# noahares/raxtax

Hardware: AMD Instinct MI355X
Metric: classified queries/sec (whole node) (higher is better)
Workload: dtype u32 bit-planes + f64

## Files before the change

include/raxtax_hip.h:

```cpp
#ifndef RAXTAX_HIP_H
#define RAXTAX_HIP_H

#include <stddef.h>
#include <stdint.h>

#ifdef __cplusplus
extern "C" {
#endif

#define RTX_ABI_VERSION 6
#define RTX_NUM_KMERS 65536u
#define RTX_MAX_DEPTH 32u

#define RTX_OK 0
#define RTX_ERR_INVALID (-1)
#define RTX_ERR_HIP (-2)
#define RTX_ERR_NO_DEVICE (-3)
#define RTX_ERR_OOM (-4)
#define RTX_ERR_PARSE (-5)
#define RTX_ERR_DEPTH (-6)
#define RTX_ERR_STATE (-7)
#define RTX_ERR_TOO_LONG (-8)
#define RTX_ERR_SENDER (-9)
#define RTX_RETRY_CHUNK 1

#define RTX_SKIP_EXACT_MATCHES 1u
#define RTX_RAW_CONFIDENCE 2u
#define RTX_TEXT_TSV 4u

#define RTX_Q_OK 0
#define RTX_Q_NO_KMERS 1

#define RTX_Q_ALL_KMERS 2

typedef struct rtx_tree rtx_tree;
typedef struct rtx_index rtx_index;

int rtx_abi_version(void);
const char *rtx_last_error(void);
int rtx_device_count(void);

int rtx_tree_build(uint64_t n, const char *lineage_bytes, const uint64_t *lineage_off,
                   const uint8_t *seq_bytes, const uint64_t *seq_off, rtx_tree **out);
#define RTX_TREE_SKIP_KMER_MAP 1u
int rtx_tree_build_ex(uint64_t n, const char *lineage_bytes, const uint64_t *lineage_off,
                      const uint8_t *seq_bytes, const uint64_t *seq_off, uint32_t flags, rtx_tree **out);
int rtx_tree_parse_reference_fasta(const char *text, uint64_t len, rtx_tree **out);
int rtx_tree_parse_reference_fasta_ex(const char *text, uint64_t len, uint32_t flags, rtx_tree **out);
int rtx_tree_build_kmer_map(rtx_tree *tree);
int rtx_tree_save_bin(const rtx_tree *tree, const char *path);
int rtx_tree_load_bin(const char *path, rtx_tree **out);
void rtx_tree_destroy(rtx_tree *tree);
uint64_t rtx_tree_num_tips(const rtx_tree *tree);
const char *rtx_tree_lineage(const rtx_tree *tree, uint64_t i);
uint64_t rtx_tree_original_index(const rtx_tree *tree, uint64_t i);
int rtx_tree_kmer_csr(const rtx_tree *tree, const uint64_t **offsets, const uint32_t **postings);
uint64_t rtx_tree_exact_matches(const rtx_tree *tree, const uint8_t *seq, uint64_t len,
                                const uint32_t **ids);
uint64_t rtx_tree_exact_matches_batch(const rtx_tree *tree, uint64_t n_queries, const uint8_t *bases,
                                      const uint64_t *base_off, uint64_t *exact_off, uint32_t *exact_ids,
                                      uint64_t ids_cap);
typedef struct {
    uint32_t n_nodes;
    const uint32_t *node_begin;
    const uint32_t *node_end;
    const uint32_t *node_first_child;
    const uint32_t *node_n_children;
    const uint32_t *node_parent;
    const uint8_t *node_type;
} rtx_nodes_view;
int rtx_tree_nodes(const rtx_tree *tree, rtx_nodes_view *out);

typedef struct rtx_queries rtx_queries;
int rtx_queries_parse_fasta(const char *text, uint64_t len, const char *const *skip, uint64_t n_skip,
                            rtx_queries **out);
#define RTX_FASTA_MORE_FOLLOWS 1u
#define RTX_FASTA_NOT_FIRST 2u
uint64_t rtx_fasta_block_end(const char *text, uint64_t len);
int rtx_queries_parse_fasta_block(const char *text, uint64_t len, const char *const *skip, uint64_t n_skip, uint32_t flags,
                                  rtx_queries **out);
void rtx_queries_destroy(rtx_queries *q);
uint64_t rtx_queries_len(const rtx_queries *q);
const char *rtx_queries_label(const rtx_queries *q, uint64_t i);
int rtx_queries_data(const rtx_queries *q, const uint8_t **bases, const uint64_t **base_off);

int rtx_index_create(int device, uint64_t n_refs, const uint64_t *offsets ,
                     const uint32_t *postings, uint32_t n_nodes, const uint32_t *node_begin,
                     const uint32_t *node_end, const uint32_t *node_first_child,
                     const uint32_t *node_n_children, const uint8_t *node_type, rtx_index **out);
int rtx_index_create_shard(int device, uint64_t n_refs_total, uint64_t ref_lo, uint64_t ref_hi,
                           const uint64_t *shard_cuts, uint32_t n_cuts, const uint64_t *offsets,
                           const uint32_t *postings, uint32_t n_nodes, const uint32_t *node_begin,
                           const uint32_t *node_end, const uint32_t *node_first_child,
                           const uint32_t *node_n_children, const uint8_t *node_type, rtx_index **out);
int rtx_index_create_from_sequences(int device, uint64_t n_refs, const uint8_t *seq_bytes, const uint64_t *seq_off,
                                    uint32_t n_nodes, const uint32_t *node_begin, const uint32_t *node_end,
                                    const uint32_t *node_first_child, const uint32_t *node_n_children,
                                    const uint8_t *node_type, rtx_index **out);
int rtx_index_create_from_tree(int device, const rtx_tree *tree, rtx_index **out);
void rtx_index_destroy(rtx_index *index);
uint64_t rtx_index_num_refs(const rtx_index *index);
uint64_t rtx_index_device_bytes(const rtx_index *index);
uint64_t rtx_index_workspace_bytes(const rtx_index *index);
int rtx_index_workspace_parts(const rtx_index *index, uint64_t out[9]);
int rtx_index_set_batch(rtx_index *index, uint32_t sub_batch);
#define RTX_OPT_SUB_BATCH 1
#define RTX_OPT_PROB_MODE 2
#define RTX_OPT_STAGE_TIMING 6
#define RTX_OPT_DEBUG_TAPS 14
#define RTX_OPT_DEVICE_EXACT 15
#define RTX_OPT_CLUSTER 7
#define RTX_OPT_PACKED_COUNTS 8
#define RTX_OPT_HIT_PAIR 11
#define RTX_OPT_TILE_SKIP 10
#define RTX_OPT_LOCATOR 12
#define RTX_OPT_TILE_PRUNE 13
#define RTX_OPT_FINE_BOUNDS 17
#define RTX_OPT_RECORDS 18
#define RTX_OPT_OVERLAP 19
#define RTX_OPT_MIN_SUB_BATCHES 20
#define RTX_OPT_TWO_LEVEL_BOUNDS 21
#define RTX_OPT_PRUNE_SELF_SAMPLE 22
#define RTX_OPT_RUN_AHEAD 23
#define RTX_OPT_DEVICE_TEXT 24
#define RTX_OPT_STRAND 25
#define RTX_OPT_NEAREST 26
#define RTX_NO_REF 0xFFFFFFFFu
#define RTX_OPT_DEREP 27
int rtx_index_set_option(rtx_index *index, int option, uint64_t value);

int rtx_index_self_sample(rtx_index *index, const uint8_t *seq_bytes, const uint64_t *seq_off, uint64_t n_refs, uint32_t n_sample, double *live_fraction);
int rtx_index_prune_verdict(const rtx_index *index, int *pruning, double *live_fraction);
int rtx_index_run_ahead_stats(const rtx_index *index, uint64_t *enqueued_ahead, uint64_t *abandoned);
#define RTX_DEFAULT_SEGMENT_CLASSES 1
#define RTX_DEFAULT_EXACT_HASH_MASK 2
#define RTX_DEFAULT_DEREP_HASH_MASK 3
int rtx_set_default_option(int option, uint64_t value);

typedef struct {
    uint32_t n_queries;
    uint64_t n_rows;
    const uint32_t *t;
    const uint8_t *status;
    const double *global_signal;
    const uint64_t *row_begin;
    const uint32_t *row_count;
    const uint32_t *row_lineage;
    const uint32_t *row_node;
    const uint32_t *row_depth;
    const double *row_conf;
    const double *row_local_signal;
    uint32_t row_conf_stride;
    const uint8_t *row_depth_u8;
    const uint8_t *row_conf_hundredths;
} rtx_result_view;

int rtx_batch_prefetch(rtx_index *index, uint64_t n_queries, const uint8_t *bases, const uint64_t *base_off,
                       const uint32_t *exact_ids, const uint64_t *exact_off);
int rtx_batch_activate(rtx_index *index);
int rtx_pack_bases(const uint8_t *bases, uint64_t n_bases, uint8_t *packed);
int rtx_classify_batch(rtx_index *index, uint64_t n_queries, const uint8_t *bases,
                       const uint64_t *base_off, const uint32_t *exact_ids,
                       const uint64_t *exact_off, uint32_t flags, rtx_result_view *out);
int rtx_index_has_exact_lookup(const rtx_index *index);
int rtx_batch_exact_matches(rtx_index *index, const uint64_t **exact_off , const uint32_t **exact_ids);

int rtx_batch_strands(rtx_index *index, const uint8_t **strand, const uint32_t **peak);
int rtx_revcomp(const uint8_t *in, uint64_t n, uint8_t *out);
int rtx_batch_nearest(rtx_index *index, const uint32_t **nearest, const uint32_t **ties);
int rtx_batch_nearest_time(rtx_index *index, float *ms, uint32_t *launches);

typedef struct {
    uint32_t n_nodes;
    uint32_t cutoff_hundredths;
    uint32_t flags;
    const uint64_t *clade, *direct, *conf_sum;
    uint64_t totals[4];
} rtx_profile_view;
int rtx_index_profile_begin(rtx_index *index, uint32_t cutoff_hundredths, uint32_t flags);
int rtx_index_profile_read(rtx_index *index, rtx_profile_view *out);
int rtx_index_profile_reset(rtx_index *index);
int rtx_index_profile_end(rtx_index *index);
int rtx_index_profile_time(rtx_index *index, float *ms, uint32_t *launches);
int rtx_profile_merge(rtx_profile_view *const *views, uint32_t n, uint64_t *clade, uint64_t *direct, uint64_t *conf_sum, uint64_t totals[4]);
int64_t rtx_profile_format(const rtx_tree *tree, const uint64_t *clade, const uint64_t *direct, const uint64_t *conf_sum,
                           const uint64_t totals[4], uint32_t cutoff_hundredths, char *out, uint64_t cap);

// ... 120 lines not shown
```

raxtax_amd/_lib.py:

```python
from __future__ import annotations

import ctypes as C
from pathlib import Path

import numpy as np

PKG = Path(__file__).resolve().parent
import os as _os

LIB_PATH = Path(_os.environ.get("RTX_LIB_PATH") or PKG / "libraxtax_hip.so")

RTX_MAX_DEPTH = 32
RTX_NUM_KMERS = 65536
RTX_OK = 0
RTX_ERR_INVALID, RTX_ERR_HIP, RTX_ERR_NO_DEVICE, RTX_ERR_OOM = -1, -2, -3, -4
RTX_ERR_PARSE, RTX_ERR_DEPTH, RTX_ERR_STATE, RTX_ERR_TOO_LONG = -5, -6, -7, -8
RTX_SKIP_EXACT_MATCHES = 1
RTX_RAW_CONFIDENCE = 2
RTX_TEXT_TSV = 4
RTX_Q_OK, RTX_Q_NO_KMERS, RTX_Q_ALL_KMERS = 0, 1, 2
RTX_OPT_DEREP = 27
RTX_DEFAULT_DEREP_HASH_MASK = 3
STAGES = ("kmer_extract", "hit_count", "prob_table", "taxon_prefix", "lineage_walk", "tile_bounds", "tile_prune", "exact_match", "order", "pair_union")

# ... 3 lines not shown
u64p = C.POINTER(C.c_uint64)
f64p = C.POINTER(C.c_double)
f32p = C.POINTER(C.c_float)


class NodesView(C.Structure):
    _fields_ = [("n_nodes", C.c_uint32), ("node_begin", u32p), ("node_end", u32p), ("node_first_child", u32p),
                ("node_n_children", u32p), ("node_parent", u32p), ("node_type", u8p)]


class ResultView(C.Structure):
    _fields_ = [("n_queries", C.c_uint32), ("n_rows", C.c_uint64), ("t", u32p), ("status", u8p),
                ("global_signal", f64p), ("row_begin", u64p), ("row_count", u32p), ("row_lineage", u32p), ("row_node", u32p),
                ("row_depth", u32p), ("row_conf", f64p), ("row_local_signal", f64p),
                ("row_conf_stride", C.c_uint32), ("row_depth_u8", u8p), ("row_conf_hundredths", u8p)]


class TextView(C.Structure):
    _fields_ = [("n_queries", C.c_uint64), ("out", C.c_void_p), ("out_off", u64p), ("tsv", C.c_void_p), ("tsv_off", u64p)]


class ProfileView(C.Structure):
    _fields_ = [("n_nodes", C.c_uint32), ("cutoff_hundredths", C.c_uint32), ("flags", C.c_uint32), ("clade", u64p), ("direct", u64p),
                ("conf_sum", u64p), ("totals", C.c_uint64 * 4)]


class RtxError(RuntimeError):
    def __init__(self, code: int, msg: str):
        super().__init__(f"libraxtax_hip error {code}: {msg}")
        self.code = code


_SIGNATURES = {
    "rtx_abi_version": (C.c_int, []),
    "rtx_last_error": (C.c_char_p, []),
    "rtx_device_count": (C.c_int, []),
    "rtx_tree_build": (C.c_int, [C.c_uint64, C.c_char_p, u64p, u8p, u64p, C.POINTER(C.c_void_p)]),
    "rtx_tree_build_ex": (C.c_int, [C.c_uint64, C.c_char_p, u64p, u8p, u64p, C.c_uint32, C.POINTER(C.c_void_p)]),
    "rtx_tree_parse_reference_fasta": (C.c_int, [C.c_char_p, C.c_uint64, C.POINTER(C.c_void_p)]),
    "rtx_tree_parse_reference_fasta_ex": (C.c_int, [C.c_char_p, C.c_uint64, C.c_uint32, C.POINTER(C.c_void_p)]),
    "rtx_tree_build_kmer_map": (C.c_int, [C.c_void_p]),
    "rtx_tree_save_bin": (C.c_int, [C.c_void_p, C.c_char_p]),
    "rtx_tree_load_bin": (C.c_int, [C.c_char_p, C.POINTER(C.c_void_p)]),
    "rtx_tree_destroy": (None, [C.c_void_p]),
    "rtx_tree_num_tips": (C.c_uint64, [C.c_void_p]),
    "rtx_tree_lineage": (C.c_char_p, [C.c_void_p, C.c_uint64]),
    "rtx_tree_original_index": (C.c_uint64, [C.c_void_p, C.c_uint64]),
    "rtx_tree_kmer_csr": (C.c_int, [C.c_void_p, C.POINTER(u64p), C.POINTER(u32p)]),
    "rtx_tree_exact_matches": (C.c_uint64, [C.c_void_p, u8p, C.c_uint64, C.POINTER(u32p)]),
    "rtx_tree_exact_matches_batch": (C.c_uint64, [C.c_void_p, C.c_uint64, u8p, u64p, u64p, u32p, C.c_uint64]),
    "rtx_tree_nodes": (C.c_int, [C.c_void_p, C.POINTER(NodesView)]),
    "rtx_fasta_block_end": (C.c_uint64, [C.c_char_p, C.c_uint64]),
    "rtx_queries_parse_fasta_block": (C.c_int, [C.c_char_p, C.c_uint64, C.POINTER(C.c_char_p), C.c_uint64, C.c_uint32,
                                      C.POINTER(C.c_void_p)]),
    "rtx_queries_parse_fasta": (C.c_int, [C.c_char_p, C.c_uint64, C.POINTER(C.c_char_p), C.c_uint64,
                                          C.POINTER(C.c_void_p)]),
    "rtx_queries_destroy": (None, [C.c_void_p]),
    "rtx_queries_len": (C.c_uint64, [C.c_void_p]),
    "rtx_queries_label": (C.c_char_p, [C.c_void_p, C.c_uint64]),
    "rtx_queries_data": (C.c_int, [C.c_void_p, C.POINTER(u8p), C.POINTER(u64p)]),
    "rtx_index_create": (C.c_int, [C.c_int, C.c_uint64, u64p, u32p, C.c_uint32, u32p, u32p, u32p, u32p, u8p,
                                   C.POINTER(C.c_void_p)]),
    "rtx_index_create_shard": (C.c_int, [C.c_int, C.c_uint64, C.c_uint64, C.c_uint64, u64p, C.c_uint32, u64p, u32p, C.c_uint32,
                                        u32p, u32p, u32p, u32p, u8p, C.POINTER(C.c_void_p)]),
    "rtx_shard_begin": (C.c_int, [C.c_void_p, u32p, u32p]),
    "rtx_shard_count": (C.c_int, [C.c_void_p, C.c_uint32, C.c_uint32]),
    "rtx_shard_bounds": (C.c_int, [C.c_void_p, C.c_uint32, C.c_uint32]),
    "rtx_shard_prunes": (C.c_int, [C.c_void_p]),
    "rtx_shard_prob": (C.c_int, [C.c_void_p, C.c_uint32]),
    "rtx_shard_walk": (C.c_int, [C.c_void_p, C.c_uint32, C.c_void_p]),
    "rtx_shard_info": (C.c_int, [C.c_void_p, u64p, u64p, u32p, u32p, u32p]),
    "rtx_device_buffer": (C.c_int, [C.c_void_p, C.c_int, C.POINTER(C.c_void_p), u64p]),
    "rtx_shard_buffer": (C.c_int, [C.c_void_p, C.c_uint32, C.c_int, C.POINTER(C.c_void_p), u64p]),
    "rtx_shard_rehist": (C.c_int, [C.c_void_p, C.c_uint32]),
    "rtx_index_stream": (C.c_int, [C.c_void_p, C.POINTER(C.c_void_p)]),
    "rtx_index_create_from_sequences": (C.c_int, [C.c_int, C.c_uint64, u8p, u64p, C.c_uint32, u32p, u32p, u32p, u32p, u8p,
                                                 C.POINTER(C.c_void_p)]),
    "rtx_index_create_from_tree": (C.c_int, [C.c_int, C.c_void_p, C.POINTER(C.c_void_p)]),
    "rtx_index_destroy": (None, [C.c_void_p]),
    "rtx_index_num_refs": (C.c_uint64, [C.c_void_p]),
    "rtx_index_device_bytes": (C.c_uint64, [C.c_void_p]),
    "rtx_index_workspace_bytes": (C.c_uint64, [C.c_void_p]),
    "rtx_index_workspace_parts": (C.c_int, [C.c_void_p, u64p]),
    "rtx_index_set_batch": (C.c_int, [C.c_void_p, C.c_uint32]),
    "rtx_set_default_option": (C.c_int, [C.c_int, C.c_uint64]),
    "rtx_index_set_option": (C.c_int, [C.c_void_p, C.c_int, C.c_uint64]),
    "rtx_index_self_sample": (C.c_int, [C.c_void_p, C.c_void_p, C.c_void_p, C.c_uint64, C.c_uint32, C.POINTER(C.c_double)]),
    "rtx_index_prune_verdict": (C.c_int, [C.c_void_p, C.POINTER(C.c_int), C.POINTER(C.c_double)]),
    "rtx_index_run_ahead_stats": (C.c_int, [C.c_void_p, C.POINTER(C.c_uint64), C.POINTER(C.c_uint64)]),
    "rtx_classify_batch": (C.c_int, [C.c_void_p, C.c_uint64, u8p, u64p, u32p, u64p, C.c_uint32,
                                     C.POINTER(ResultView)]),
    "rtx_index_has_exact_lookup": (C.c_int, [C.c_void_p]),
    "rtx_batch_exact_matches": (C.c_int, [C.c_void_p, C.POINTER(u64p), C.POINTER(u32p)]),
    "rtx_batch_upload": (C.c_int, [C.c_void_p, C.c_uint64, u8p, u64p, u32p, u64p]),
    "rtx_batch_run": (C.c_int, [C.c_void_p, C.c_uint32]),
    "rtx_batch_sync": (C.c_int, [C.c_void_p]),
    "rtx_batch_download": (C.c_int, [C.c_void_p, C.POINTER(ResultView)]),
    "rtx_batch_download_then_run": (C.c_int, [C.c_void_p, C.POINTER(ResultView), C.c_uint32]),
    "rtx_index_text_setup": (C.c_int, [C.c_void_p, C.c_void_p, C.c_uint32]),
    "rtx_batch_prefetch_labels": (C.c_int, [C.c_void_p, C.c_uint64, C.POINTER(C.c_char_p)]),
    "rtx_batch_text": (C.c_int, [C.c_void_p, C.POINTER(TextView)]),
    "rtx_batch_stage_times": (C.c_int, [C.c_void_p, f32p, u32p]),
    "rtx_batch_work": (C.c_int, [C.c_void_p, u64p, u64p, u64p]),
    "rtx_batch_prob_work": (C.c_int, [C.c_void_p, u64p, u64p]),
    "rtx_batch_work_split": (C.c_int, [C.c_void_p, u64p, u64p]),
    "rtx_debug_kmers": (C.c_int, [C.c_void_p, C.c_uint64, u16p, u32p]),
    "rtx_debug_hit_counts": (C.c_int, [C.c_void_p, C.c_uint64, u16p]),
    "rtx_debug_prob_table": (C.c_int, [C.c_void_p, C.c_uint64, f64p, f64p]),
    "rtx_debug_pruned_prob_table": (C.c_int, [C.c_void_p, C.c_uint64, f64p, f64p, u32p]),
    "rtx_debug_probs": (C.c_int, [C.c_void_p, C.c_uint64, f64p]),
    "rtx_debug_order": (C.c_int, [C.c_void_p, u32p]),
    "rtx_debug_tile_bounds": (C.c_int, [C.c_void_p, C.c_uint64, u16p]),
    "rtx_debug_prune_stats": (C.c_int, [C.c_void_p, u64p]),
    "rtx_debug_run_counts": (C.c_int, [C.c_void_p, C.c_uint64, u16p, u8p, u32p, u32p, u32p]),
    "rtx_debug_run_mode": (C.c_int, [C.c_void_p, C.c_uint64, u32p]),
    "rtx_batch_last_sub_batch": (C.c_int, [C.c_void_p, u64p, u32p]),
    "rtx_batch_classes": (C.c_int, [C.c_void_p, u32p, u64p]),
    "rtx_debug_prune_detail": (C.c_int, [C.c_void_p, C.c_uint64, u32p]),
    "rtx_debug_evaluate": (C.c_int, [C.c_void_p, f64p, C.POINTER(ResultView)]),
    "rtx_result_pack": (C.c_int64, [C.POINTER(ResultView), u8p, C.c_uint64]),
    "rtx_records_format": (C.c_int64, [C.c_void_p, u8p, C.c_uint64, C.POINTER(C.c_char_p), u32p, C.c_uint32, C.c_char_p, C.c_uint64, u64p, C.c_uint32]),
    "rtx_format_query": (C.c_int64, [C.c_void_p, C.POINTER(ResultView), C.c_uint64, C.c_char_p, u8p, C.c_uint64,
                                     u32p, C.c_uint64, C.c_uint32, C.c_char_p, C.c_uint64, C.c_char_p, C.c_uint64,
                                     C.POINTER(C.c_int64)]),
    "rtx_raxtax": (C.c_int, None),
    "rtx_raxtax_multi": (C.c_int, None),
    "rtx_raxtax_multi_ex": (C.c_int, None),
    "rtx_batch_strands": (C.c_int, [C.c_void_p, C.POINTER(u8p), C.POINTER(u32p)]),
    "rtx_revcomp": (C.c_int, [u8p, C.c_uint64, u8p]),
    "rtx_raxtax_multi_ex2": (C.c_int, None),
    "rtx_batch_nearest": (C.c_int, [C.c_void_p, C.POINTER(u32p), C.POINTER(u32p)]),
    "rtx_batch_nearest_time": (C.c_int, [C.c_void_p, C.POINTER(C.c_float), C.POINTER(C.c_uint32)]),
    "rtx_index_profile_begin": (C.c_int, [C.c_void_p, C.c_uint32, C.c_uint32]),
    "rtx_index_profile_read": (C.c_int, [C.c_void_p, C.POINTER(ProfileView)]),
    "rtx_index_profile_reset": (C.c_int, [C.c_void_p]),
    "rtx_index_profile_end": (C.c_int, [C.c_void_p]),
    "rtx_index_profile_time": (C.c_int, [C.c_void_p, C.POINTER(C.c_float), C.POINTER(C.c_uint32)]),
    "rtx_profile_merge": (C.c_int, [C.POINTER(C.POINTER(ProfileView)), C.c_uint32, u64p, u64p, u64p, u64p]),
    "rtx_profile_format": (C.c_int64, [C.c_void_p, u64p, u64p, u64p, u64p, C.c_uint32, C.c_char_p, C.c_uint64]),
    "rtx_batch_prefetch_weights": (C.c_int, [C.c_void_p, C.c_uint64, u32p]),
    "rtx_derep_create": (C.c_int, [C.c_int, C.POINTER(C.c_void_p)]),
    "rtx_derep_run": (C.c_int, [C.c_void_p, C.c_uint64, u8p, u64p, u32p, C.POINTER(C.c_uint64)]),
    "rtx_derep_destroy": (None, [C.c_void_p]),
    "rtx_derep_plan": (C.c_int, [C.c_uint64, u32p, u32p, u32p, u32p, C.POINTER(C.c_uint64)]),
    "rtx_raxtax_last_derep": (C.c_int, [C.POINTER(C.c_uint64), C.POINTER(C.c_uint64), C.POINTER(C.c_double)]),
    "rtx_sender_discard": (C.c_int, [C.c_void_p, C.c_char_p, C.c_char_p, C.c_char_p]),
    "rtx_batch_prefetch": (C.c_int, [C.c_void_p, C.c_uint64, u8p, u64p, u32p, u64p]),
    "rtx_batch_activate": (C.c_int, [C.c_void_p]),
    "rtx_pack_bases": (C.c_int, [u8p, C.c_uint64, u8p]),
    "rtx_batch_sub_batch": (C.c_int, [C.c_void_p, C.POINTER(C.c_uint32), C.POINTER(C.c_uint32)]),
    "rtx_raxtax_last_timing": (C.c_int, [C.POINTER(C.c_double), C.POINTER(C.c_uint64)]),
    "rtx_set_host_share": (C.c_int, [C.c_uint32]),
    "rtx_host_threads": (C.c_uint32, []),
}

_lib = None


def load() -> C.CDLL:
    global _lib
    if _lib is not None:
        return _lib
    if not LIB_PATH.exists():
        raise ImportError(
            f"{LIB_PATH} is missing: build it with `python -m raxtax_amd._build` (hipcc, gfx950). "
            "raxtax_amd has no CPU fallback.")
# ... 23 lines not shown
```

raxtax_amd/api.py:

```python
from __future__ import annotations

import ctypes as C
from dataclasses import dataclass
from typing import Callable, List, Optional, Sequence, Tuple

import numpy as np

from . import _lib
from ._lib import (RTX_MAX_DEPTH, RTX_RAW_CONFIDENCE, RTX_SKIP_EXACT_MATCHES, NodesView, ResultView, RtxError, check,
                   f32p, f64p, ptr, u8p, u16p, u32p, u64p)


def _flatten(seqs: Sequence[np.ndarray]) -> Tuple[np.ndarray, np.ndarray]:
    off = np.zeros(len(seqs) + 1, dtype=np.uint64)
    if len(seqs):
        off[1:] = np.cumsum([len(s) for s in seqs], dtype=np.uint64)
    flat = np.zeros(max(int(off[-1]), 1), dtype=np.uint8)
    for i, s in enumerate(seqs):
        flat[int(off[i]):int(off[i + 1])] = np.asarray(s, dtype=np.uint8)
    return flat, off


class Tree:

# ... 127 lines not shown
    node: int
    confidence_values: List[float]
    local_signal: float
    global_signal: float


class Result:

    def __init__(self, view: ResultView, strand: Optional[np.ndarray] = None, peak: Optional[np.ndarray] = None,
                 nearest: Optional[np.ndarray] = None, nearest_ties: Optional[np.ndarray] = None):
        nq, nr = view.n_queries, view.n_rows
        self.strand, self.peak = strand, peak
        self.nearest, self.nearest_ties = nearest, nearest_ties
        arr = lambda p, n: (np.ctypeslib.as_array(p, shape=(n,)).copy() if n else np.zeros(0))
        self.n_queries = nq
        self.t = arr(view.t, nq)
        self.status = arr(view.status, nq)
        self.global_signal = arr(view.global_signal, nq)
        begin = arr(view.row_begin, nq).astype(np.int64)
        count = arr(view.row_count, nq).astype(np.int64)
        self.row_off = np.zeros(nq + 1, dtype=np.uint64)
        self.row_off[1:] = np.cumsum(count)
        src = (np.repeat(begin - self.row_off[:-1].astype(np.int64), count) + np.arange(int(count.sum()))) if nq else np.zeros(0, np.int64)
        assert len(src) <= nr
        self.row_lineage = arr(view.row_lineage, nr)[src]
        self.row_node = arr(view.row_node, nr)[src]
        self.row_depth = arr(view.row_depth, nr)[src]
        stride = int(view.row_conf_stride) or RTX_MAX_DEPTH
        self.row_conf = (np.ctypeslib.as_array(view.row_conf, shape=(nr, stride))[src] if nr
                         else np.zeros((0, stride)))
        self.row_local_signal = arr(view.row_local_signal, nr)[src]
        self.row_conf_hundredths = (np.ctypeslib.as_array(view.row_conf_hundredths, shape=(nr, stride))[src].copy() if nr and view.row_conf_hundredths
                                    else np.rint(self.row_conf * 100.0).astype(np.uint8))

    def rows(self, q: int) -> List[EvaluationResult]:
        out = []
        for r in range(int(self.row_off[q]), int(self.row_off[q + 1])):
            d = int(self.row_depth[r])
            out.append(EvaluationResult(int(self.row_lineage[r]), int(self.row_node[r]),
                                        [float(x) for x in self.row_conf[r, :d]],
                                        float(self.row_local_signal[r]), float(self.global_signal[q])))
        return out


@dataclass
class Profile:
    cutoff: int
    flags: int
    clade: np.ndarray
    direct: np.ndarray
    conf_sum: np.ndarray
    totals: np.ndarray

    def _view(self) -> "_lib.ProfileView":
        v = _lib.ProfileView()
        v.n_nodes, v.cutoff_hundredths, v.flags = len(self.clade), self.cutoff, self.flags
        v.clade, v.direct, v.conf_sum = ptr(self.clade, u64p), ptr(self.direct, u64p), ptr(self.conf_sum, u64p)
        for i in range(4):
            v.totals[i] = int(self.totals[i])
        return v


def profile_merge(profiles: Sequence[Profile]) -> Profile:
    if not profiles:
        raise ValueError("profile_merge: no profiles")
    views = [p._view() for p in profiles]
    arr = (C.POINTER(_lib.ProfileView) * len(views))(*[C.pointer(v) for v in views])
    n = len(profiles[0].clade)
    clade, direct, conf = (np.zeros(n, np.uint64) for _ in range(3))
    totals = np.zeros(4, np.uint64)
    check(_lib.load().rtx_profile_merge(arr, len(views), ptr(clade, u64p), ptr(direct, u64p), ptr(conf, u64p), ptr(totals, u64p)))
    return Profile(profiles[0].cutoff, profiles[0].flags, clade, direct, conf, totals)


def profile_text(tree: Tree, profile: Profile) -> str:
    lib = _lib.load()
    a = [np.ascontiguousarray(x, dtype=np.uint64) for x in (profile.clade, profile.direct, profile.conf_sum, profile.totals)]
    args = [tree._h] + [ptr(x, u64p) for x in a] + [int(profile.cutoff)]
    n = check(lib.rtx_profile_format(*args, None, 0))
    buf = C.create_string_buffer(max(n, 1))
    check(lib.rtx_profile_format(*args, buf, n))
    return buf.raw[:n].decode()


DEFAULT_SEGMENT_CLASSES = 1


class Index:

    nearest_on = False

    def __init__(self, tree: Tree, device: int = 0, sub_batch: int = 0, prob_mode: int = 0,
                 stage_timing: bool = False, cluster: Optional[bool] = None, segment_classes=None,
                 packed_counts: Optional[bool] = None,
                 tile_skip: Optional[bool] = None, hit_pair=None, locator: Optional[bool] = None, tile_prune: Optional[bool] = None,
                 debug_taps: bool = False, device_exact: Optional[bool] = None, fine_bounds: Optional[bool] = None,
                 records: Optional[int] = None, overlap: Optional[bool] = None, two_level: Optional[int] = None,
                 prune_self_sample: Optional[bool] = None, device_text: bool = False, strand: str = "plus",
                 nearest: bool = False, derep: bool = False):
        self._lib = _lib.load()
        self.tree = tree
        if segment_classes is None:
            segment_classes = DEFAULT_SEGMENT_CLASSES
        check(self._lib.rtx_set_default_option(1, int(segment_classes)))
        h = C.c_void_p()
        check(self._lib.rtx_index_create_from_tree(device, tree._h, C.byref(h)))
        self._h = h
        self.n_refs = self._lib.rtx_index_num_refs(self._h)
        if sub_batch:
            check(self._lib.rtx_index_set_batch(self._h, sub_batch))
        if prob_mode:
            check(self._lib.rtx_index_set_option(self._h, 2, prob_mode))
        if stage_timing:
            check(self._lib.rtx_index_set_option(self._h, 6, 1))
        if cluster is not None:
            check(self._lib.rtx_index_set_option(self._h, 7, int(cluster)))
        if packed_counts is not None:
            check(self._lib.rtx_index_set_option(self._h, 8, int(packed_counts)))
        if tile_skip is not None:
            check(self._lib.rtx_index_set_option(self._h, 10, int(tile_skip)))
        if hit_pair is not None:
            check(self._lib.rtx_index_set_option(self._h, 11, int(hit_pair)))
        if locator is not None:
            check(self._lib.rtx_index_set_option(self._h, 12, int(locator)))
        if tile_prune is not None:
            check(self._lib.rtx_index_set_option(self._h, 13, int(tile_prune)))
            if tile_prune and prune_self_sample is None:
                check(self._lib.rtx_index_set_option(self._h, 22, 0))
        if debug_taps:
            check(self._lib.rtx_index_set_option(self._h, 14, 1))
        if device_exact is not None:
            check(self._lib.rtx_index_set_option(self._h, 15, int(device_exact)))
        if device_text:
            check(self._lib.rtx_index_set_option(self._h, 24, 1))
        if fine_bounds is not None:
            check(self._lib.rtx_index_set_option(self._h, 17, int(fine_bounds)))
        if records is not None:
            check(self._lib.rtx_index_set_option(self._h, 18, int(records)))
        if overlap is not None:
            check(self._lib.rtx_index_set_option(self._h, 19, int(overlap)))
        if two_level is not None:
            check(self._lib.rtx_index_set_option(self._h, 21, int(two_level)))
        if prune_self_sample is not None:
            check(self._lib.rtx_index_set_option(self._h, 22, int(prune_self_sample)))
        if strand not in ("plus", "both"):
            raise ValueError(f"strand must be 'plus' or 'both', not {strand!r}")
        self.strand = strand
        if strand == "both":
            check(self._lib.rtx_index_set_option(self._h, 25, 1))
        self.nearest_on = bool(nearest)
        if nearest:
            check(self._lib.rtx_index_set_option(self._h, 26, 1))
        if derep:
            check(self._lib.rtx_index_set_option(self._h, _lib.RTX_OPT_DEREP, 1))
        self._view = ResultView()
        self._keep = None

    @property
    def prune_verdict(self):
        on, frac = C.c_int(), C.c_double()
        check(self._lib.rtx_index_prune_verdict(self._h, C.byref(on), C.byref(frac)))
        return bool(on.value), float(frac.value)

    @property
    def run_ahead_stats(self):
        a, b = C.c_uint64(), C.c_uint64()
        check(self._lib.rtx_index_run_ahead_stats(self._h, C.byref(a), C.byref(b)))
        return int(a.value), int(b.value)

    def __del__(self):
        try:
            if self._h:
                self._lib.rtx_index_destroy(self._h)
                self._h = None
        except Exception:
            pass

    @property
    def device_bytes(self) -> int:
        return self._lib.rtx_index_device_bytes(self._h)

    @property
    def workspace_bytes(self) -> int:
        return self._lib.rtx_index_workspace_bytes(self._h)

    def workspace_parts(self) -> dict:
        out = np.zeros(9, dtype=np.uint64)
        check(self._lib.rtx_index_workspace_parts(self._h, ptr(out, u64p)))
        names = ("prob_tables", "counts", "record_segments", "prefix_sums", "tile_masks_and_slot_lists", "other_scratch", "inputs_and_order", "results")
        d = {k: int(v) for k, v in zip(names, out[:8])}
        d["scratch_sets"] = int(out[8])
        return d

    def upload(self, bases: np.ndarray, base_off: np.ndarray, exact_ids: Optional[np.ndarray] = None,
               exact_off: Optional[np.ndarray] = None):
        self.prefetch(bases, base_off, exact_ids, exact_off)
        self.activate()

    def prefetch(self, bases: np.ndarray, base_off: np.ndarray, exact_ids: Optional[np.ndarray] = None,
                 exact_off: Optional[np.ndarray] = None):
        bases = np.ascontiguousarray(bases, dtype=np.uint8)
        base_off = np.ascontiguousarray(base_off, dtype=np.uint64)
        n_q = len(base_off) - 1
        if exact_off is not None:
            exact_off = np.ascontiguousarray(exact_off, dtype=np.uint64)
            exact_ids = np.ascontiguousarray(exact_ids if exact_ids is not None and len(exact_ids) else
                                             np.zeros(1, np.uint32), dtype=np.uint32)
            check(self._lib.rtx_batch_prefetch(self._h, n_q, ptr(bases, u8p), ptr(base_off, u64p), ptr(exact_ids, u32p),
                                               ptr(exact_off, u64p)))
        else:
            check(self._lib.rtx_batch_prefetch(self._h, n_q, ptr(bases, u8p), ptr(base_off, u64p), None, None))

    def prefetch_weights(self, weights: np.ndarray):
        w = np.ascontiguousarray(weights, dtype=np.uint32)
        check(self._lib.rtx_batch_prefetch_weights(self._h, len(w), ptr(w if len(w) else np.zeros(1, np.uint32), u32p)))

    def activate(self):
        check(self._lib.rtx_batch_activate(self._h))

    def run(self, flags: int = 0):
        check(self._lib.rtx_batch_run(self._h, flags))

    def sync(self):
        check(self._lib.rtx_batch_sync(self._h))

    def download(self, copy: bool = True):
        check(self._lib.rtx_batch_download(self._h, C.byref(self._view)))
        return Result(self._view, *self.strands(), *(self.nearest() if self.nearest_on else (None, None))) if copy else self._view

    def nearest(self):
        pn, pt = u32p(), u32p()
        check(self._lib.rtx_batch_nearest(self._h, C.byref(pn), C.byref(pt)))
        n = self._view.n_queries
        if not n:
            return np.zeros(0, np.uint32), np.zeros(0, np.uint32)
        return np.ctypeslib.as_array(pn, shape=(n,)).copy(), np.ctypeslib.as_array(pt, shape=(n,)).copy()

    def nearest_time(self):
        ms, n = C.c_float(), C.c_uint32()
        check(self._lib.rtx_batch_nearest_time(self._h, C.byref(ms), C.byref(n)))
        return float(ms.value), int(n.value)

    def profile_begin(self, cutoff: float = 0.8, skip_exact_matches: bool = False, raw_confidence: bool = False):
        flags = (RTX_SKIP_EXACT_MATCHES if skip_exact_matches else 0) | (RTX_RAW_CONFIDENCE if raw_confidence else 0)
        check(self._lib.rtx_index_profile_begin(self._h, int(round(cutoff * 100)), flags))

    def profile_read(self) -> Profile:
        v = _lib.ProfileView()
        check(self._lib.rtx_index_profile_read(self._h, C.byref(v)))
        n = v.n_nodes
        g = lambda p: np.ctypeslib.as_array(p, shape=(n,)).copy() if n else np.zeros(0, np.uint64)
        return Profile(int(v.cutoff_hundredths), int(v.flags), g(v.clade), g(v.direct), g(v.conf_sum), np.array(list(v.totals), dtype=np.uint64))

    def profile_reset(self):
        check(self._lib.rtx_index_profile_reset(self._h))

    def profile_end(self):
        check(self._lib.rtx_index_profile_end(self._h))

    def profile_time(self):
        ms, n = C.c_float(), C.c_uint32()
        check(self._lib.rtx_index_profile_time(self._h, C.byref(ms), C.byref(n)))
        return float(ms.value), int(n.value)

    def strands(self):
        ps, pk = u8p(), u32p()
        check(self._lib.rtx_batch_strands(self._h, C.byref(ps), C.byref(pk)))
        n = self._view.n_queries
# ... 303 lines not shown
```

raxtax_amd/csrc/rtx_api_batch.hip:

```cpp
#include "rtx_index.hpp"

#ifndef RTX_B2_HEAVY_PER_ATILE
#define RTX_B2_HEAVY_PER_ATILE 4u
#endif

namespace rtxi {

int bind(rtx_index *ix) {
    if (!ix) { set_error("null index handle"); return RTX_ERR_INVALID; }
    RTX_HIP(hipSetDevice(ix->device));
    return RTX_OK;
}

int ensure_events(rtx_index *ix, size_t count) {
    while (ix->events.size() < count) {
        hipEvent_t e;
        RTX_HIP(hipEventCreate(&e));
        ix->events.push_back(e);
    }
    return RTX_OK;
}


SubBatch sub_batch_of(rtx_index *ix, uint32_t sb, bool timed) {
// ... 144 lines not shown
    up.n_refs = ix->u_nblocks;
    up.dmask = nullptr;
    up.nsparse = nullptr;
    up.ntiles = ix->u_ntiles;
    up.counts = nullptr;
    up.counts_lo = nullptr;
    up.counts_hi = nullptr;
    up.hist = nullptr;
    up.tile_max = nullptr;
    up.bounds_tile_ub = sc.d_tile_ub.p;
    up.bounds_tile_stride = ix->ntiles;
    up.bounds_ntiles = ix->ntiles;
    up.bounds_best = sc.d_best_key.p;
    up.flags = 0;
    up.group_base = hp.group_base + ix->n_groups_run;
    return up;
}

static Bounds2Params bounds2_params(const rtx_index *ix, const rtx_index::Scratch &sc, const HitParams &up, bool heavy) {
    Bounds2Params bp{};
    bp.abitmap = ix->d_abitmap.p;
    bp.bbitmap = ix->d_bbitmap.p;
    bp.n_rows1 = ix->n_rows + 1;
    bp.n_atiles = ix->n_atiles;
    bp.ntiles = ix->ntiles;
    bp.zero_row = ix->n_rows;
    bp.pair_urec = sc.d_urec.p;
    bp.pair_nu = sc.d_nu.p;
    bp.pair_ustride = up.pair_ustride;
    bp.nq = up.nq;
    bp.t = sc.d_t.p;
    bp.tile_ub = sc.d_tile_ub.p;
    bp.tile_ub_stride = ix->ntiles;
    bp.best_key = sc.d_best_key.p;
    bp.delta_ct = ix->b2_delta[0];
    bp.delta_cm = ix->b2_delta[1];
    bp.delta_lo = ix->b2_delta[2];
    bp.delta_hi = ix->b2_delta[3];
    bp.group_rows = up.group_rows;
    bp.group_base = up.group_base;
    bp.heavy = heavy ? sc.d_heavy.p : nullptr;
    bp.heavy_max = std::max<uint32_t>(1u, std::min<uint32_t>(RTX_B2_HEAVY_PER_ATILE * ix->n_atiles, ix->n_btiles / 2u));
    return bp;
}

static PruneParams prune_params(rtx_index *ix, const SubBatch &b, uint32_t flags, int part, const ExactRef &exact) {
    rtx_index::Scratch &sc = ix->sc[b.set];
    const rtx_index::BatchClass &k = *b.cls;
    PruneParams pr{};
    pr.tile_ub = sc.d_tile_ub.p;
    pr.best_key = sc.d_best_key.p;
    pr.tile_ub_stride = ix->ntiles;
    pr.ntiles = ix->ntiles;
    pr.nq = b.nq;
    pr.n_refs = ix->n_refs;
    pr.n_total = ix->n_total;
    pr.ref_base = ix->ref_lo;
    pr.phase = (uint32_t)part;
    pr.best = part ? sc.d_best.p : nullptr;
    pr.bitmap = ix->d_bitmap.p;
    pr.cbitmap = part == 0 && (ix->two_level_used || (k.planes > kBounds2MaxPlanes && ix->two_level_opt && ix->n_refs == ix->n_total)) ? reinterpret_cast<const uint2 *>(ix->d_cbitmap.p) : nullptr;
    pr.n_rows1 = ix->n_rows + 1;
    pr.stride_bytes = ix->stride_bytes;
    pr.rows = sc.d_rows.p;
    pr.rstride = k.rstride;
    pr.nrows = sc.d_nrows.p;
    pr.t = sc.d_t.p;
    pr.flags = flags;
    pr.q0 = b.q0;
    pr.perm = ix->res().d_perm.p;
    pr.exact = exact;
    pr.lnfact = ix->d_lnfact.p;
    pr.inv = ix->d_inv.p;
    pr.nlf = std::min<uint32_t>(kLnFactLen, k.tmax + k.tmax / 2 + 2);
    pr.hist = sc.d_hist.p;
    pr.hstride = k.hstride;
    pr.live = sc.d_live.p;
    pr.live_words = LiveLayout{ix->ntiles}.words();
    pr.pair_live = ItemsLayout(b.nq, ix->ntiles).pair_live(sc.d_items.p);
    pr.thr_out = sc.d_prune_thr.p;
    pr.i1_out = sc.d_prune_i1.p;
    pr.stats = ix->d_prune_stats.p;
    pr.detail = ix->debug_taps && ix->d_prune_detail.n >= (size_t)b.nq * kPruneDetailWords ? ix->d_prune_detail.p : nullptr;
    return pr;
}

static HitParams fine_params(const rtx_index *ix, const rtx_index::Scratch &sc, const HitParams &hp) {
    HitParams fp = hp;
    fp.bitmap = ix->d_fbitmap.p;
    fp.stride_bytes = ix->f_stride_bytes;
    fp.n_refs = ix->f_nblocks;
    fp.ntiles = ix->f_ntiles;
    fp.counts = nullptr;
    fp.counts_lo = nullptr;
    fp.counts_hi = nullptr;
    fp.tile_max = nullptr;
    fp.flags = 0;
    fp.group_rows = nullptr;
    fp.live = sc.d_live.p;
    fp.live_words = LiveLayout{ix->ntiles}.words();
    fp.prune_thr = sc.d_prune_thr.p;
    fp.fine_n_refs = ix->n_refs;
    fp.fine_ref_ntiles = ix->ntiles;
    fp.fine_stats = ix->d_prune_stats.p + 2 * kPruneStatCopies * 8;
    return fp;
}

int enqueue_hit(rtx_index *ix, const SubBatch &b, uint32_t flags, hipStream_t s, int part, hipStream_t s_mid) {
    rtx_index::Scratch &sc = ix->sc[b.set];
    rtx_index::ResultSet &r = ix->res();
    const rtx_index::BatchClass &k = *b.cls;
    ix->last_set = b.set;
    HitParams hp = hit_params(ix, b, flags);
    const bool prune = run_prunes(ix, k);
    if (k.pair && part != 2) {
        if (b.timed_all) RTX_HIP(hipEventRecord(stage_event(ix, b, RTX_STAGE_PAIR_UNION, 0), s));
        launch_pair_union(s, sc.d_rows.p, sc.d_nrows.p, k.rstride, b.nq, sc.d_urec.p, sc.d_nu.p, 2u * k.rstride);
        if (b.timed_all) RTX_HIP(hipEventRecord(stage_event(ix, b, RTX_STAGE_PAIR_UNION, 1), s));
    }
    if (b.timed && !prune) RTX_HIP(hipEventRecord(stage_event(ix, b, RTX_STAGE_HIT_COUNT, 0), s));
    if (part != 0 && !prune) { set_error("internal: a split run without tile pruning"); return RTX_ERR_STATE; }
    if (prune) {
        if (part != 2) {
            const HitParams up = bounds_params(ix, sc, hp);
            if (b.timed) RTX_HIP(hipEventRecord(stage_event(ix, b, RTX_STAGE_TILE_BOUNDS, 0), s));
            ix->two_level_used = part == 0 && ix->two_level_opt && ix->d_abitmap.p && ix->d_bbitmap.p && ix->n_refs == ix->n_total && k.planes <= kBounds2MaxPlanes;
            if (ix->two_level_used) {
                const bool heavy_ok = sc.d_heavy.p && sc.d_heavy_items.p && sc.d_heavy_items.n >= HeavyItemsLayout(b.nq, ix->u_ntiles).total();
                launch_bounds2(s, bounds2_params(ix, sc, up, heavy_ok), b.nq, k.planes, up, ix->u_ntiles, heavy_ok ? sc.d_heavy_items.p : nullptr);
            } else {
                RTX_HIP(hipMemsetAsync(sc.d_best_key.p, 0, (size_t)b.nq * 4, s));
                launch_hit_count_pair_bounds(s, up, b.nq, ix->u_ntiles, k.planes);
            }
            if (b.timed) RTX_HIP(hipEventRecord(stage_event(ix, b, RTX_STAGE_TILE_BOUNDS, 1), s));
        }
        if (s_mid && s_mid != s && part == 0) {
            RTX_HIP(hipEventRecord(ix->ev_mid[b.sb], s));
            RTX_HIP(hipStreamWaitEvent(s_mid, ix->ev_mid[b.sb], 0));
            s = s_mid;
        }
        if (b.timed && part != 1) RTX_HIP(hipEventRecord(stage_event(ix, b, RTX_STAGE_TILE_PRUNE, 0), s));
        PruneParams pr = prune_params(ix, b, flags, part, hp.exact);
        const bool records = part == 0 && on_records_path(ix, k, sc), diet = part == 0 && on_diet(ix, k, sc);
        const RecordRef rr = record_ref(ix, sc, r);
        if (records) { pr.rec = rr; pr.rec_max_slots = rr.stride; }
        if (k.diet && !diet) { set_error("internal: the counts buffer is on its diet without the records path"); return RTX_ERR_STATE; }
        if (diet) {
            RTX_HIP(hipMemsetAsync(sc.d_cnt_cursor.p, 0, 4, s));
            pr.cnt_row = sc.d_cnt_row.p;
            pr.cnt_cursor = sc.d_cnt_cursor.p;
            pr.cnt_cap = k.cnt_rows;
            pr.flags_out = r.d_flags.p;
            hp.cnt_row = sc.d_cnt_row.p;
        }
        launch_prune(s, pr, prob_tables(ix), b.nq);
        if (part == 1) { RTX_HIP(hipGetLastError()); return RTX_OK; }
        if (part == 0 && ix->fine_opt && ix->d_fbitmap.p && k.pair && sc.d_fine_items.p) {
            const FineItemsLayout fine(b.nq, ix->f_ntiles);
            uint32_t *const fi = sc.d_fine_items.p;
            launch_fine_bounds(s, fine_params(ix, sc, hp), b.nq, ix->ntiles, ix->f_ntiles, pr.pair_live, fine.cursors(fi), fine.items(fi), fine.count(fi), k.planes);
        }
        RTX_HIP(hipMemsetAsync(sc.d_tilemax.p, 0, (size_t)b.nq * ix->ntiles * 2, s));
        hp.live = sc.d_live.p;
        hp.live_words = pr.live_words;
        hp.prune_thr = sc.d_prune_thr.p;
        if (records) hp.rec = rr;
        if (k.pair) {
            const ItemsLayout items(b.nq, ix->ntiles);
            launch_live_items(s, sc.d_live.p, pr.live_words, pr.pair_live, b.nq, ix->ntiles, items.offsets(sc.d_items.p), items.items(sc.d_items.p), items.count(sc.d_items.p));
            hp.items = items.items(sc.d_items.p);
            hp.n_items = items.count(sc.d_items.p);
        }
        if (ix->seg_blocks) {
            KmerParams kp = kmer_params(ix, b);
            kp.mode = 2u;
            kp.live = sc.d_live.p;
            kp.live_words = pr.live_words;
            launch_kmer_extract(s, kp, b.nq);
        }
        if (b.timed) {
            RTX_HIP(hipEventRecord(stage_event(ix, b, RTX_STAGE_TILE_PRUNE, 1), s));
            RTX_HIP(hipEventRecord(stage_event(ix, b, RTX_STAGE_HIT_COUNT, 0), s));
        }
    }
    if (k.pair) launch_hit_count_pair(s, hp, b.nq, ix->ntiles, k.planes);
    else launch_hit_count(s, hp, b.nq, ix->ntiles, k.planes);
    if (b.timed) RTX_HIP(hipEventRecord(stage_event(ix, b, RTX_STAGE_HIT_COUNT, 1), s));
    ix->hit_stream = s;
    return RTX_OK;
}

int enqueue_count(rtx_index *ix, const SubBatch &b, uint32_t flags, hipStream_t s_mid) {
    int rc = enqueue_kmer(ix, b, b.s);
    return rc ? rc : enqueue_hit(ix, b, flags, b.s, 0, s_mid);
}

static WalkParams walk_params(rtx_index *ix, const SubBatch &b, const double *prefix);
static int reset_sub_alloc(rtx_index *ix, hipStream_t s);

int enqueue_prob_prefix(rtx_index *ix, const SubBatch &b, bool fuse_walk, bool prob_only) {
    rtx_index::Scratch &sc = ix->sc[b.set];
    const rtx_index::BatchClass &k = *b.cls;
    hipStream_t s = b.s;
    ProbParams pp{};
    pp.t = sc.d_t.p;
    pp.hist = sc.d_hist.p;
    pp.hstride = k.hstride;
    pp.tmax = k.tmax;
    pp.n1max = k.tmax / 2 + 1;
    pp.lnfact = ix->d_lnfact.p;
    pp.n_refs = ix->n_total;
    pp.q0 = b.q0;
    pp.table_z = sc.d_table_z.p;
    rtx_index::ResultSet &r = ix->res();
    pp.z = r.d_z.p;
    pp.gs = r.d_gs.p;
    pp.status = r.d_status.p;
    pp.ndist = r.d_ndist.p;
    pp.prune_thr = run_prunes(ix, k) ? sc.d_prune_thr.p : nullptr;
    pp.prune_i1 = pp.prune_thr ? sc.d_prune_i1.p : nullptr;
    if (b.timed_all) RTX_HIP(hipEventRecord(stage_event(ix, b, RTX_STAGE_PROB_TABLE, 0), s));
    if (k.use_tables) {
        launch_prob_order(s, sc.d_t.p, b.nq, sc.d_order.p);
        pp.order = sc.d_order.p;
        launch_prob_lookup(s, pp, prob_tables(ix), b.nq);
    } else {
        if (k.huge) {
            pp.gstride = (uint32_t)((prob_table_lds_bytes(k.tmax) + 7) / 8);
            if (ix->d_prob_scratch.n < (size_t)b.nq * pp.gstride) { set_error("internal: scratch of prob_table too small"); return RTX_ERR_STATE; }
            pp.gscratch = ix->d_prob_scratch.p;
        }
        launch_prob_table(s, pp, b.nq);
    }
    if (b.timed_all) RTX_HIP(hipEventRecord(stage_event(ix, b, RTX_STAGE_PROB_TABLE, 1), s));
    if (prob_only) return RTX_OK;

    PrefixParams fp{};
    fp.status = r.d_status.p;
    fp.t = sc.d_t.p;
    fp.tz_in_lds = (size_t)k.hstride * 8 <= 16 * 1024 ? 1u : 0u;
    fp.q0 = b.q0;
    fp.counts = sc.d_counts.p;
    fp.counts_lo = counts_lo(ix, sc);
    fp.counts_hi = counts_hi(ix, k, sc);
    fp.packed = ix->packs(k.planes) ? 1u : 0u;
    fp.npad = ix->npad;
    fp.table_z = sc.d_table_z.p;
    fp.hstride = k.hstride;
    fp.n_refs = ix->n_refs;
    fp.bnd_bits = ix->d_bnd_bits.p;
    fp.bnd_rank = ix->d_bnd_rank.p;
    fp.prefix = sc.d_prefix.p;
    fp.n_bnd = ix->n_bnd_local;
    fp.tile_max = ix->tile_skip ? sc.d_tilemax.p : nullptr;
    fp.ntiles = ix->ntiles;
    fp.prune_thr = pp.prune_thr;
    fp.prune_stats = fp.prune_thr ? ix->d_prune_stats.p + kPruneStatCopies * 8 : nullptr;
    fp.fuse_walk = fuse_walk ? 1u : 0u;
    const bool records = fuse_walk && on_records_path(ix, k, sc);
    fp.rec_nslots = records ? sc.d_rec_nslots.p : nullptr;
    fp.cnt_row = fuse_walk && on_diet(ix, k, sc) ? sc.d_cnt_row.p : nullptr;
    if (fuse_walk) {
        fp.walk = walk_params(ix, b, sc.d_prefix.p);
        int rc_r = fp.walk.sub_alloc ? reset_sub_alloc(ix, s) : RTX_OK;
        if (rc_r) return rc_r;
    }
    if (b.timed_all) RTX_HIP(hipEventRecord(stage_event(ix, b, RTX_STAGE_TAXON_PREFIX, 0), s));
    launch_taxon_prefix(s, fp, b.nq);
    if (records) {
        TailParams tp{};
        tp.rec = record_ref(ix, sc, r);
        tp.t = sc.d_t.p;
        tp.table_z = sc.d_table_z.p;
        tp.hstride = k.hstride;
        tp.bnd_bits = ix->d_bnd_bits.p;
        tp.bnd_rank = ix->d_bnd_rank.p;
        tp.prefix = sc.d_prefix.p;
        if (fp.cnt_row) { tp.cnt_cursor = sc.d_cnt_cursor.p; tp.cnt_cap = k.cnt_rows; tp.flags_out = r.d_flags.p; }
        tp.n_bnd = ix->n_bnd_local;
        tp.nq = b.nq;
        tp.walk = fp.walk;
        tp.prefix_stats = fp.prune_stats;
        tp.stats = ix->d_prune_stats.p ? ix->d_prune_stats.p + 3 * kPruneStatCopies * 8 : nullptr;
        launch_records_tail(s, tp, b.nq);
    }
    if (b.timed_all) RTX_HIP(hipEventRecord(stage_event(ix, b, RTX_STAGE_TAXON_PREFIX, 1), s));
    return RTX_OK;
}

int alloc_result_set(rtx_index *ix, rtx_index::ResultSet &r, uint64_t n_queries, uint64_t min_arena) {
    int rc;
    if ((rc = r.d_status.alloc(n_queries)) || (rc = r.d_t_all.alloc(n_queries)) || (rc = r.d_nrows_all.alloc(n_queries)) ||
        (rc = r.d_n_rows.alloc(n_queries)) || (rc = r.d_gs.alloc(n_queries)) || (rc = r.d_z.alloc(n_queries)) ||
        (rc = r.d_hq.alloc(n_queries)) || (rc = r.d_row_start.alloc(n_queries)) || (rc = r.d_ndist.alloc(n_queries)) ||
        (rc = r.d_cursor.alloc(2)) || (rc = r.d_flags.alloc(1)))
        return rc;
    const uint64_t want_arena = std::max<uint64_t>(n_queries * 10 + 4096, min_arena);
    if (r.arena_cap < want_arena) {
        if ((rc = r.d_arena.alloc(want_arena))) return rc;
        r.arena_cap = want_arena;
    }
    return alloc_final(ix, r, n_queries);
}

int settle_join(rtx_index *ix) {
    if (ix->join_pending && ix->join_ev) RTX_HIP(hipStreamWaitEvent(ix->stream, ix->join_ev, 0));
    ix->join_pending = false;
    return RTX_OK;
}

int alloc_final(rtx_index *ix, rtx_index::ResultSet &r, uint64_t n_queries) {
    int rc;
    if ((rc = r.d_fin_t.alloc(n_queries)) || (rc = r.d_fin_status.alloc(n_queries)) || (rc = r.d_fin_gs.alloc(n_queries)) ||
        (rc = r.d_fin_row_begin.alloc(n_queries)) || (rc = r.d_fin_row_count.alloc(n_queries)) || (rc = r.d_fin_cursor.alloc(2)))
        return rc;
    if ((rc = r.d_peak2.alloc(n_queries)) || (rc = r.d_peak.alloc(n_queries)) || (rc = r.d_strand.alloc(n_queries))) return rc;
    if (ix->nearest_opt && ((rc = r.d_nearest2.alloc(n_queries)) || (rc = r.d_ties2.alloc(n_queries)) || (rc = r.d_nearest.alloc(n_queries)) || (rc = r.d_ties.alloc(n_queries))))
        return rc;
    if (ix->strand_opt && ((rc = r.d_sel_t.alloc(n_queries)) || (rc = r.d_sel_status.alloc(n_queries)) || (rc = r.d_sel_gs.alloc(n_queries)) ||
                           (rc = r.d_sel_row_begin.alloc(n_queries)) || (rc = r.d_sel_row_count.alloc(n_queries))))
        return rc;
    const uint64_t rows = r.arena_cap, D = ix->fin_D;
    if ((rc = r.d_fin_lineage.alloc(rows)) || (rc = r.d_fin_node.alloc(rows)) || (rc = r.d_fin_depth.alloc(rows)) || (rc = r.d_fin_depth8.alloc(rows)) ||
        (rc = r.d_fin_local.alloc(rows)) || (rc = r.d_fin_conf.alloc(rows * D)) || (rc = r.d_fin_hund.alloc(rows * D)))
        return rc;
    r.fin_cap = rows;
    return RTX_OK;
}

int enqueue_finalise(rtx_index *ix, const SubBatch &b, hipStream_t s) {
    rtx_index::ResultSet &r = ix->res();
    FinaliseParams fp{};
    fp.status = r.d_status.p;
    fp.t_all = r.d_t_all.p;
    fp.gs = r.d_gs.p;
    fp.n_rows = r.d_n_rows.p;
    fp.row_start = r.d_row_start.p;
    fp.arena = r.d_arena.p;
    fp.arena_cap = r.arena_cap;
    fp.perm = r.d_perm.p;
    fp.q0 = b.q0;
    fp.nq = b.nq;
    fp.node_depth = ix->d_node_depth.p;
    fp.node_sig0 = ix->d_node_sig0.p;
    fp.node_begin = ix->d_node_begin.p;
    fp.node_eb = ix->d_node_eb.p;
    fp.D = ix->fin_D;
    fp.o_t = r.d_fin_t.p;
    fp.o_status = r.d_fin_status.p;
    fp.o_gs = r.d_fin_gs.p;
    fp.o_row_begin = r.d_fin_row_begin.p;
    fp.o_row_count = r.d_fin_row_count.p;
    fp.r_lineage = r.d_fin_lineage.p;
    fp.r_node = r.d_fin_node.p;
    fp.r_depth = r.d_fin_depth.p;
// ... 536 lines not shown
    uint32_t n_sets = ix->n_refs == ix->n_total && !ix->shared_device ? 1u + std::min<uint32_t>(ix->overlap_opt, 2u) : 1u;
    size_t free_b = 0, total_b = 0;
    RTX_HIP(hipMemGetInfo(&free_b, &total_b));
    uint64_t held = 0;
    for (const auto &sc : ix->sc) held += sc.d_counts.n * 2 + sc.d_prefix.n * 8 + sc.d_rec.n * 4 + sc.d_srows.n * 4;
    const uint64_t budget = (uint64_t)((free_b + held) * 0.6);
    uint64_t worst = 0;
    for (uint32_t c = 0; c < ix->n_cls; c++) {
        rtx_index::BatchClass &k = ix->cls[c];
        k.will_prune = ix->pruning() && ix->d_ubitmap.p && ix->pair_opt && ix->ntiles >= RTX_PRUNE_MIN_TILES && k.tmax <= kProbTablesMaxT && (ix->n_refs == ix->n_total || ix->shard_prune_opt);
        const uint64_t per_q = class_per_q(ix, k);
        uint32_t B = ix->sub_batch_req;
        if (B == 0) {
            B = (uint32_t)std::min<uint64_t>(k.will_prune ? kDefaultSubBatchPruned : ix->ntiles >= 16 ? kDefaultSubBatchLarge : kDefaultSubBatch,
                                             std::max<uint64_t>(64, budget / per_q));
            if (k.huge) B = std::min<uint32_t>(B, 1024u);
            if (k.will_prune && k.n < (uint64_t)ix->min_subs * B) B = (uint32_t)std::max<uint64_t>(16384, (k.n + ix->min_subs - 1) / ix->min_subs);
        }
        if (B > kMaxSubBatch) B = kMaxSubBatch;
        B = (uint32_t)std::max<uint64_t>(1, std::min<uint64_t>(B, k.n));
        k.sub_batch = B;
        worst = std::max<uint64_t>(worst, (uint64_t)B * per_q);
    }
    {
        uint32_t bulk = 0;
        for (uint32_t c = 1; c < ix->n_cls; c++)
            if (ix->cls[c].n > ix->cls[bulk].n) bulk = c;
        worst = 0;
        for (uint32_t c = 0; c < ix->n_cls; c++) {
            ix->cls[c].side = ix->n_refs == ix->n_total && c != bulk && ix->cls[c].n <= kSideMaxQueries && ix->cls[c].n * 64u <= ix->cls[bulk].n;
            if (!ix->cls[c].side) worst = std::max<uint64_t>(worst, (uint64_t)ix->cls[c].sub_batch * class_per_q(ix, ix->cls[c]));
        }
    }
    {
        uint64_t n_side_q = 0;
        for (uint32_t c = 0; c < ix->n_cls; c++)
            if (ix->cls[c].side) n_side_q += ix->cls[c].n;
        const uint64_t want2 = want_arena + (n_side_q ? n_side_q * kWalkMaxRows + 64 : 0);
        if (r.arena_cap < want2) {
            if ((rc = r.d_arena.alloc(want2))) return rc;
            r.arena_cap = want2;
        }
    }
    while (n_sets > 1u && (uint64_t)n_sets * worst > budget) n_sets--;
    ix->staged = false;
    if ((rc = plan_sub_batches(ix))) return rc;
    if ((rc = alloc_scratch_set(ix, 0))) return rc;
    {
        bool any_side = false;
        for (uint32_t c = 0; c < ix->n_cls; c++) any_side = any_side || ix->cls[c].side;
        if (any_side) { if ((rc = alloc_scratch_set(ix, kSideSet))) return rc; }
        else ix->sc[kSideSet].release_all();
    }
    for (uint32_t k = 1; k <= 2u; k++) {
        if (k < n_sets && ix->n_sub_total() > 1) {
            if (alloc_scratch_set(ix, k)) ix->sc[k].d_kmers.release();
        } else if (ix->n_refs == ix->n_total) {
            ix->sc[k].release_all();
        }
    }
    return RTX_OK;
}

int alloc_scratch_set(rtx_index *ix, uint32_t k) {
    int rc;
    rtx_index::Scratch &sc = ix->sc[k];
    const ScratchNeed n = scratch_set_need(ix, k);
    if ((rc = sc.d_kmers.alloc(n.kmers)) || (rc = sc.d_rows.alloc(n.rows)) || (rc = sc.d_dmask.alloc(n.dmask)) || (rc = sc.d_nsparse.alloc(n.nsparse)) || (rc = sc.d_srows.alloc(n.srows)) ||
        (rc = sc.d_t.alloc(n.t)) || (rc = sc.d_nrows.alloc(n.nrows)) || (rc = sc.d_counts.alloc(n.counts)) || (rc = sc.d_hist.alloc(n.hist)) || (rc = sc.d_table_z.alloc(n.hist)) ||
        (rc = sc.d_prefix.alloc(n.prefix)) || (rc = sc.d_order.alloc(n.order)) || (rc = sc.d_tilemax.alloc(n.tilemax)) || (rc = sc.d_urec.alloc(n.urec)) || (rc = sc.d_nu.alloc(n.nu)))
        return rc;
    if (n.prob_scratch && (rc = ix->d_prob_scratch.alloc(std::max(n.prob_scratch, ix->d_prob_scratch.n)))) return rc;
    if (ix->pruning() && ix->d_ubitmap.p && (ix->n_refs == ix->n_total || ix->shard_prune_opt)) {
        if ((rc = sc.d_tile_ub.alloc(n.tile_ub)) || (rc = sc.d_best_key.alloc(n.best_key)) || (rc = sc.d_prune_thr.alloc(n.prune_thr)) || (rc = sc.d_prune_i1.alloc(n.prune_i1)) ||
            (rc = sc.d_best.alloc(n.best)) || (rc = sc.d_live.alloc(n.live)) || (rc = sc.d_items.alloc(n.items)))
            return rc;
        if (ix->d_abitmap.p && (sc.d_heavy.alloc(n.heavy) || sc.d_heavy_items.alloc(n.heavy_items))) { sc.d_heavy.release(); sc.d_heavy_items.release(); }
        if (ix->d_fbitmap.p && sc.d_fine_items.alloc(n.fine_items)) sc.d_fine_items.release();
        if (ix->rec_opt && ix->n_refs == ix->n_total) {
            if (sc.d_rec_nslots.alloc(n.rec_nslots) || sc.d_rec_slots.alloc(n.rec_slots) || sc.d_rec_cnt.alloc(n.rec_cnt) ||
                sc.d_rec.alloc(n.rec) || sc.d_cnt_row.alloc(n.cnt_row) || sc.d_cnt_cursor.alloc(n.cnt_cursor))
                sc.d_rec.release();
        }
    }
    return RTX_OK;
}

}

extern "C" {

int rtx_batch_prefetch(rtx_index *ix, uint64_t n_queries, const uint8_t *bases, const uint64_t *base_off,
                       const uint32_t *exact_ids, const uint64_t *exact_off) {
    int rc = bind(ix);
    if (rc) return rc;
    rtx_index::Inputs &in = ix->in[ix->cur_in ^ 1u];
    const bool with_labels = in.labels_pending && in.n_labels == n_queries;
    in.labels_pending = in.has_labels = false;
    const bool with_weights = in.weights_pending && in.n_weights == n_queries;
    in.weights_pending = in.has_weights = false;
    if (n_queries == 0 || !base_off || (!bases && base_off[n_queries])) {
        set_error("rtx_batch_upload: invalid argument");
        return RTX_ERR_INVALID;
    }
    const bool both = ix->strand_opt != 0u;
    if (both) {
        if (exact_off || exact_ids) { set_error("RTX_OPT_STRAND: exact-match ids cannot be passed in (those of the reverse complements must come from the same lookup: pass NULL)"); return RTX_ERR_INVALID; }
        if (!rtx_index_has_exact_lookup(ix) || ix->n_refs != ix->n_total) { set_error("RTX_OPT_STRAND needs the exact-match lookup of the device (a handle built from the reference sequences, RTX_OPT_DEVICE_EXACT on)"); return RTX_ERR_STATE; }
        if (n_queries > 0x7FFFFFFFull) { set_error("RTX_OPT_STRAND: too many queries in one batch"); return RTX_ERR_INVALID; }
    }
    const uint64_t n_dev = both ? 2 * n_queries : n_queries;
    if (!ix->h2d_stream) RTX_HIP(hipStreamCreateWithFlags(&ix->h2d_stream, hipStreamNonBlocking));
    if (!in.ready) RTX_HIP(hipEventCreateWithFlags(&in.ready, hipEventDisableTiming));
    if (in.recorded) RTX_HIP(hipEventSynchronize(in.ready));
    in.staged = false;
    if (ix->ev_activated) RTX_HIP(hipStreamWaitEvent(ix->h2d_stream, ix->ev_activated, 0));
    uint64_t max_len = 0;
    uint64_t cls_n[5] = {0, 0, 0, 0, 0}, cls_max[5] = {0, 0, 0, 0, 0};
    {
        const uint64_t lim3 = class3_max_len();
        for (uint64_t q = 0; q < n_queries; q++) {
            if (base_off[q + 1] < base_off[q]) { set_error("base_off not monotone at query %llu", (unsigned long long)q); return RTX_ERR_INVALID; }
            const uint64_t len = base_off[q + 1] - base_off[q];
            max_len = std::max(max_len, len);
            const int c = len <= 262 ? 0 : (len <= 1030 ? 1 : (len <= kMidClassMaxT + 7 ? 2 : (len <= lim3 ? 3 : 4)));
            cls_n[c]++;
            cls_max[c] = std::max(cls_max[c], len);
        }
    }
    const uint64_t total = base_off[n_queries] - base_off[0];
    uint64_t n_exact = 0;
    if (exact_off) {
        if (exact_off[0] != 0) { set_error("exact_off[0] must be 0"); return RTX_ERR_INVALID; }
        n_exact = exact_off[n_queries];
        for (uint64_t q = 0; q < n_queries; q++)
            if (exact_off[q + 1] < exact_off[q]) { set_error("exact_off not monotone"); return RTX_ERR_INVALID; }
        if (n_exact && !exact_ids) { set_error("exact_ids is null"); return RTX_ERR_INVALID; }
        for (uint64_t i = 0; i < n_exact; i++)
            if (exact_ids[i] >= ix->n_total) { set_error("exact id %u out of range", exact_ids[i]); return RTX_ERR_INVALID; }
    }
    const uint64_t n_packed = (total + 1) / 2;
    if ((rc = in.h_packed.resize(total + 64)) || (rc = in.h_base_off.resize(n_queries + 1)) || (rc = in.d_packed.alloc(total + 64)) ||
        (rc = in.d_base_off.alloc(n_dev + 1)) || (rc = in.d_exact_off.alloc(n_dev + 1)) || (rc = in.d_exact_ids.alloc(n_exact + 1)))
        return rc;
    for (uint64_t q = 0; q <= n_queries; q++) in.h_base_off[q] = base_off[q] - base_off[0];
    in.packed = total == 0 || rtx::pack_nibbles_mt(bases + base_off[0], total, in.h_packed.data(), rtx::host_threads(8u));
    if (!in.packed) std::memcpy(in.h_packed.data(), bases + base_off[0], total);
    RTX_HIP(hipMemcpyAsync(in.d_packed.p, in.h_packed.data(), in.packed ? n_packed : total, hipMemcpyHostToDevice, ix->h2d_stream));
    RTX_HIP(hipMemcpyAsync(in.d_base_off.p, in.h_base_off.data(), (n_queries + 1) * 8, hipMemcpyHostToDevice, ix->h2d_stream));
    if (exact_off) {
        if ((rc = in.h_exact_off.resize(n_queries + 1)) || (rc = in.h_exact_ids.resize(n_exact + 1))) return rc;
        std::memcpy(in.h_exact_off.data(), exact_off, (n_queries + 1) * 8);
        if (n_exact) std::memcpy(in.h_exact_ids.data(), exact_ids, n_exact * 4);
        RTX_HIP(hipMemcpyAsync(in.d_exact_off.p, in.h_exact_off.data(), (n_queries + 1) * 8, hipMemcpyHostToDevice, ix->h2d_stream));
        if (n_exact) RTX_HIP(hipMemcpyAsync(in.d_exact_ids.p, in.h_exact_ids.data(), n_exact * 4, hipMemcpyHostToDevice, ix->h2d_stream));
    } else {
        RTX_HIP(hipMemsetAsync(in.d_exact_off.p, 0, (n_dev + 1) * 8, ix->h2d_stream));
    }
    RTX_HIP(hipEventRecord(in.ready, ix->h2d_stream));
    in.recorded = true;
    in.n_q = n_dev;
    in.n_user = n_queries;
    in.total = total;
    in.max_len = max_len;
    for (int c = 0; c < 5; c++) { in.cls_n[c] = both ? 2 * cls_n[c] : cls_n[c]; in.cls_max[c] = cls_max[c]; }
    in.n_exact = n_exact;
// ... 76 lines not shown
```

raxtax_amd/csrc/rtx_api_index.hip:

```cpp
#include "rtx_index.hpp"

namespace rtx {
int index_device(const rtx_index *index) { return index ? index->device : -1; }
void index_set_shared_device(rtx_index *index, bool shared) { if (index) index->shared_device = shared; }
uint32_t index_swap_min_subs(rtx_index *index, uint32_t v) { if (!index) return 0; const uint32_t old = index->min_subs; index->min_subs = v; return old; }
bool index_strand(const rtx_index *index) { return index && index->strand_opt != 0u; }
bool index_nearest(const rtx_index *index) { return index && index->nearest_opt != 0u; }
bool index_profile(const rtx_index *index, uint32_t *cutoff_hundredths, uint32_t *flags) {
    if (!index || !index->prof.on) return false;
    if (cutoff_hundredths) *cutoff_hundredths = index->prof.cutoff;
    if (flags) *flags = index->prof.flags;
    return true;
}
bool index_device_text(const rtx_index *index) { return index && index->device_text_opt != 0u; }
bool index_derep(const rtx_index *index) { return index && index->derep_opt != 0u; }
uint32_t index_swap_run_ahead(rtx_index *index, uint32_t v) {
    if (!index) return 0;
    const uint32_t old = index->run_ahead_opt;
    (void)rtx_index_set_option(index, RTX_OPT_RUN_AHEAD, v);
    return old;
}
}

namespace {
// ... 596 lines not shown
    if (bases.empty()) return RTX_OK;
    const uint32_t prune_was = ix->prune_opt, taps_was = ix->debug_taps;
    ix->prune_opt = 1u;
    ix->debug_taps = 0u;
    uint64_t st[16] = {0};
    int rc = rtx_batch_upload(ix, n, bases.data(), off.data(), nullptr, nullptr);
    if (rc == RTX_OK) rc = rtx_batch_run(ix, RTX_SKIP_EXACT_MATCHES);
    if (rc == RTX_OK) rc = rtx_batch_sync(ix);
    if (rc == RTX_OK) rc = rtx_debug_prune_stats(ix, st);
    ix->prune_opt = prune_was;
    ix->debug_taps = taps_was;
    ix->uploaded = ix->ran = ix->synced = false;
    if (rc != RTX_OK) return RTX_OK;
    if (st[5] != 0) {
        ix->self_live = (double)st[7] / ((double)st[5] * (double)ix->ntiles);
        ix->prune_pays = ix->self_live < kSelfSampleOff;
    }
    if (live_fraction) *live_fraction = ix->self_live;
    return RTX_OK;
}
int rtx_index_prune_verdict(const rtx_index *ix, int *pruning, double *live_fraction) {
    if (!ix) { set_error("null index handle"); return RTX_ERR_INVALID; }
    if (pruning) *pruning = ix->pruning() ? 1 : 0;
    if (live_fraction) *live_fraction = ix->self_live;
    return RTX_OK;
}

int rtx_index_run_ahead_stats(const rtx_index *ix, uint64_t *enqueued_ahead, uint64_t *abandoned) {
    if (!ix) { set_error("null index handle"); return RTX_ERR_INVALID; }
    if (enqueued_ahead) *enqueued_ahead = ix->n_run_ahead;
    if (abandoned) *abandoned = ix->n_run_ahead_retry;
    return RTX_OK;
}

void rtx_index_destroy(rtx_index *index) {
    if (!index) return;
    (void)hipSetDevice(index->device);
    delete index;
}

uint64_t rtx_index_num_refs(const rtx_index *index) { return index ? index->n_total : 0; }
uint64_t rtx_index_device_bytes(const rtx_index *index) {
    if (!index) return 0;
    return index->d_seg_dbits.n * 8 + index->d_seg_sbits.n * 8 + index->d_seg_sbase.n * 4 + index->d_seginfo.n * 4 + index->d_segcls.n * 4 + index->d_segslots.n * 2 + index->d_bitmap.n * 4 + index->d_row_of.n * 4 + index->d_row_len.n * 8 + index->d_list_len.n * 4 + index->d_loc_table.n * 4 + index->d_ubitmap.n * 4 + index->d_fbitmap.n * 4 + index->d_abitmap.n * 4 + index->d_bbitmap.n + index->d_cbitmap.n + index->d_em_table.n * 8 + index->d_em_rep_off.n * 8 + index->d_em_rep_bytes.n + index->d_em_goff.n * 4 + index->d_em_gids.n * 4 + index->d_lnfact.n * 8 +
           index->d_noderec.n * 16 + index->d_bnd_bits.n + index->d_bnd_rank.n * 4;
}
uint64_t rtx_index_workspace_bytes(const rtx_index *ix) {
    if (!ix) return 0;
    uint64_t b = (ix->d_tab_cmf.n + ix->d_tab_ratio.n) * 8 + ix->d_tab_off.n * 8 + ix->d_tab_moff.n * 4 + (ix->d_tab_ilo.n + ix->d_tab_sat.n) * 2 + ix->d_node_depth.n + ix->d_node_sig0.n + ix->d_node_begin.n * 4 + ix->d_node_eb.n * 8;
    for (const auto &sc : ix->sc) b += sc.bytes();
    for (const auto &in : ix->in) b += in.d_packed.n + (in.d_base_off.n + in.d_exact_off.n) * 8 + in.d_exact_ids.n * 4;
    b += ix->d_bases.n + ix->d_prob_scratch.n * 8 + (ix->d_skey_in.n + ix->d_skey_out.n) * 8 + ix->d_sidx.n * 4 + ix->d_sort_tmp.n + ix->d_group_rows.n * 4;
    for (const auto &r : ix->rs) {
        const rtx_index::ResultSet::Bytes s = r.bytes();
        b += s.order + s.groups + s.rest;
    }
    return b;
}
int rtx_index_workspace_parts(const rtx_index *ix, uint64_t out[9]) {
    if (!ix || !out) { set_error("null argument"); return RTX_ERR_INVALID; }
    for (int i = 0; i < 9; i++) out[i] = 0;
    out[0] = (ix->d_tab_cmf.n + ix->d_tab_ratio.n) * 8 + ix->d_tab_off.n * 8 + ix->d_tab_moff.n * 4 + (ix->d_tab_ilo.n + ix->d_tab_sat.n) * 2;
    for (const auto &sc : ix->sc) {
        if (!sc.d_kmers.p) continue;
        out[8]++;
        out[1] += sc.d_counts.bytes();
        out[2] += sc.d_rec.bytes() + sc.d_rec_cnt.bytes() + sc.d_rec_nslots.bytes() + sc.d_rec_slots.bytes();
        out[3] += sc.d_prefix.bytes();
        out[4] += sc.d_dmask.bytes() + sc.d_srows.bytes() + sc.d_nsparse.bytes();
    }
    out[6] = ix->d_bases.n + (ix->d_skey_in.n + ix->d_skey_out.n) * 8 + ix->d_sidx.n * 4 + ix->d_sort_tmp.n;
    for (const auto &in : ix->in) out[6] += in.d_packed.n + (in.d_base_off.n + in.d_exact_off.n) * 8 + in.d_exact_ids.n * 4;
    for (const auto &r : ix->rs) {
        const rtx_index::ResultSet::Bytes s = r.bytes();
        out[6] += s.order;
        out[7] += s.rest;
    }
    const uint64_t all = rtx_index_workspace_bytes(ix);
    uint64_t named = 0;
    for (int i = 0; i < 8; i++) named += out[i];
    out[5] = all > named ? all - named : 0;
    return RTX_OK;
}
int rtx_index_set_batch(rtx_index *index, uint32_t sub_batch) {
    if (!index) { set_error("null index handle"); return RTX_ERR_INVALID; }
    index->uploaded = index->ran = index->synced = false;
    index->sub_batch_req = sub_batch;
    return RTX_OK;
}

int rtx_set_default_option(int option, uint64_t value) {
    if (option == RTX_DEFAULT_SEGMENT_CLASSES) { g_seg_classes = value ? 1 : 0; return RTX_OK; }
    if (option == RTX_DEFAULT_EXACT_HASH_MASK) { g_em_hash_mask = value ? value : ~0ull; return RTX_OK; }
    if (option == RTX_DEFAULT_DEREP_HASH_MASK) { set_derep_hash_mask(value ? value : ~0ull); return RTX_OK; }
    set_error("rtx_set_default_option: unknown option %d", option);
    return RTX_ERR_INVALID;
}

int rtx_index_set_option(rtx_index *index, int option, uint64_t value) {
    if (!index) { set_error("null index handle"); return RTX_ERR_INVALID; }
    switch (option) {
        case RTX_OPT_SUB_BATCH: case RTX_OPT_PACKED_COUNTS: case RTX_OPT_HIT_PAIR: case RTX_OPT_TILE_PRUNE: case RTX_OPT_PROB_MODE:
            index->uploaded = index->ran = index->synced = false;
            break;
        default: break;
    }
    switch (option) {
        case RTX_OPT_SUB_BATCH: index->sub_batch_req = (uint32_t)value; return RTX_OK;
        case RTX_OPT_STAGE_TIMING:
            index->stage_timing = value ? 1u : 0u;
            return RTX_OK;
        case RTX_OPT_DEBUG_TAPS:
            index->debug_taps = value ? 1u : 0u;
            return RTX_OK;
        case RTX_OPT_SHARD_PRUNE:
            index->uploaded = index->ran = index->synced = false;
            index->shard_prune_opt = value ? 1u : 0u;
            return RTX_OK;
        case RTX_OPT_DEVICE_EXACT:
            index->uploaded = index->ran = index->synced = false;
            index->dev_exact_opt = value ? 1u : 0u;
            return RTX_OK;
        case RTX_OPT_CLUSTER:
            index->cluster = value ? 1u : 0u;
            return RTX_OK;
        case RTX_OPT_PACKED_COUNTS:
            index->packed_opt = value ? 1u : 0u;
            return RTX_OK;
        case RTX_OPT_HIT_PAIR:
            index->pair_opt = value ? 1u : 0u;
            return RTX_OK;
        case RTX_OPT_TILE_SKIP:
            index->tile_skip = value ? 1u : 0u;
            return RTX_OK;
        case RTX_OPT_LOCATOR:
            index->locator_opt = value ? 1u : 0u;
            return RTX_OK;
        case RTX_OPT_TILE_PRUNE:
            index->prune_opt = value ? 1u : 0u;
            return RTX_OK;
        case RTX_OPT_FINE_BOUNDS:
            index->fine_opt = value ? 1u : 0u;
            return RTX_OK;
        case RTX_OPT_PRUNE_SELF_SAMPLE:
            index->uploaded = index->ran = index->synced = false;
            index->self_sample_opt = value ? 1u : 0u;
            return RTX_OK;
        case RTX_OPT_RUN_AHEAD:
            index->run_ahead_opt = (uint32_t)std::min<uint64_t>(value, 2u);
            if (!value && index->join_pending) {
                int rc_b = bind(index);
                if (!rc_b) rc_b = settle_join(index);
                return rc_b;
            }
            return RTX_OK;
        case RTX_OPT_DEVICE_TEXT:
            index->device_text_opt = value ? 1u : 0u;
            return RTX_OK;
        case RTX_OPT_DEREP:
            if (value > 1) break;
            index->derep_opt = (uint32_t)value;
            return RTX_OK;
        case RTX_OPT_STRAND:
            if (value > 1) break;
            if (value && index->n_refs != index->n_total) { set_error("RTX_OPT_STRAND: not on a reference-shard handle (the peak of a query is spread over the shards)"); return RTX_ERR_INVALID; }
            index->uploaded = index->ran = index->synced = false;
// ... 48 lines not shown
```

raxtax_amd/csrc/rtx_index.hpp:

```cpp
#pragma once

#include <hip/hip_runtime.h>

#include <algorithm>
#include <cmath>
#include <cstdlib>
#include <cstring>
#include <thread>

#include "rtx_internal.hpp"
#include "rtx_kernels.hpp"
#include "rtx_math.hpp"

using namespace rtx;

namespace rtxi {


constexpr uint32_t kEmptyRow = 0xFFFFFFFFu;
constexpr uint32_t kLnFactLen = 98320;

#define RTX_HIP(call)                                                                          \
    do {                                                                                       \
        hipError_t e_ = (call);                                                                \
// ... 174 lines not shown
    uint32_t overlap_opt = 1;
    uint32_t overlap_used = 0;
    hipStream_t stream2 = nullptr, stream3 = nullptr, hit_stream = nullptr;
    std::vector<hipEvent_t> ev_front, ev_back, ev_mid;
    DevBuf<unsigned long long> d_prune_stats;
    uint32_t shard_prune_opt = 0;
    uint32_t debug_taps = 0;
    DevBuf<uint32_t> d_prune_detail;
    uint32_t locator_opt = 1;
    DevBuf<uint32_t> d_loc_table;
    DevBuf<uint32_t> d_group_rows;
    uint32_t n_groups_run = 0;
    uint32_t groups_per_sub = 0;
    bool packs(int pl) const { return packed_opt && pl <= 10; }
    DevBuf<uint64_t> d_skey_in, d_skey_out;
    DevBuf<uint32_t> d_sidx;
    DevBuf<uint8_t> d_sort_tmp;
    DevBuf<uint8_t> d_bases;
    struct Inputs {
        DevBuf<uint8_t> d_packed;
        DevBuf<uint64_t> d_base_off, d_exact_off;
        DevBuf<uint32_t> d_exact_ids;
        PinBuf<uint8_t> h_packed;
        PinBuf<uint64_t> h_base_off, h_exact_off;
        PinBuf<uint32_t> h_exact_ids;
        uint64_t n_q = 0, total = 0, max_len = 0, n_exact = 0;
        uint64_t n_user = 0;
        uint64_t cls_n[5] = {0, 0, 0, 0, 0}, cls_max[5] = {0, 0, 0, 0, 0};
        bool packed = true, has_exact = false, staged = false, recorded = false;
        DevBuf<char> d_labels;
        DevBuf<uint64_t> d_label_off;
        PinBuf<char> h_labels;
        PinBuf<uint64_t> h_label_off;
        uint64_t n_labels = 0;
        bool labels_pending = false, has_labels = false;
        DevBuf<uint32_t> d_weights;
        PinBuf<uint32_t> h_weights;
        uint64_t n_weights = 0;
        bool weights_pending = false, has_weights = false;
        hipEvent_t ready = nullptr;
    } in[2];
    uint32_t cur_in = 0;
    hipStream_t h2d_stream = nullptr;
    hipEvent_t ev_activated = nullptr;
    uint64_t sum_query_bytes = 0;
    uint32_t sub_batch_req = 0;
    uint32_t min_subs = 4;
    uint64_t ws_key[14] = {0};
    bool ws_valid = false;
    struct BatchClass {
        uint64_t pos0 = 0, n = 0, max_len = 0;
        uint32_t tmax = 0, kstride = 0, rstride = 0, hstride = 0, sub_batch = 0, sb0 = 0, n_sub = 0;
        int planes = 10;
        bool use_tables = false, pair = false, prune = false, rec = false, huge = false, will_prune = false;
        bool side = false;
        bool diet = false;
        uint32_t cnt_rows = 0;
    } cls[5];
    uint32_t n_cls = 0;
    uint64_t key_lim[4] = {~0ull, ~0ull, ~0ull, ~0ull};
    struct SubPlan { uint64_t q0; uint32_t nq, cls; };
    std::vector<SubPlan> plan;
    uint32_t n_sub_total() const { return (uint32_t)plan.size(); }
    uint32_t sub_batch_max = 0;
    bool any_prune = false;
    DevBuf<double> d_prob_scratch;
    struct Scratch {
        DevBuf<uint16_t> d_kmers, d_counts, d_tilemax;
        DevBuf<uint32_t> d_rows, d_t, d_nrows, d_hist, d_order, d_srows, d_nsparse;
        DevBuf<unsigned long long> d_dmask;
        DevBuf<double> d_table_z, d_prefix;
        DevBuf<uint2> d_urec;
        DevBuf<uint32_t> d_nu;
        DevBuf<uint32_t> d_live, d_best_key;
        DevBuf<uint32_t> d_items;
        DevBuf<uint16_t> d_tile_ub, d_prune_thr, d_prune_i1;
        DevBuf<uint32_t> d_best;
        DevBuf<uint8_t> d_heavy;
        DevBuf<uint32_t> d_heavy_items;
        DevBuf<uint32_t> d_fine_items;
        DevBuf<uint16_t> d_rec_nslots, d_rec_slots;
        DevBuf<uint32_t> d_rec_cnt, d_rec;
        DevBuf<uint32_t> d_cnt_row, d_cnt_cursor;
        template <class S, class F>
        static void each(S &s, F &&f) {
            f(s.d_kmers); f(s.d_counts); f(s.d_tilemax); f(s.d_rows); f(s.d_t); f(s.d_nrows); f(s.d_hist); f(s.d_order); f(s.d_srows); f(s.d_nsparse);
            f(s.d_dmask); f(s.d_table_z); f(s.d_prefix); f(s.d_urec); f(s.d_nu); f(s.d_live); f(s.d_best_key); f(s.d_items); f(s.d_tile_ub); f(s.d_prune_thr);
            f(s.d_prune_i1); f(s.d_best); f(s.d_heavy); f(s.d_heavy_items); f(s.d_fine_items); f(s.d_rec_nslots); f(s.d_rec_slots); f(s.d_rec_cnt); f(s.d_rec);
            f(s.d_cnt_row); f(s.d_cnt_cursor);
        }
        void release_all() { each(*this, [](auto &b) { b.release(); }); }
        uint64_t bytes() const {
            uint64_t b = 0;
            each(*this, [&](const auto &buf) { b += buf.bytes(); });
            return b - d_cnt_row.bytes() - d_cnt_cursor.bytes();
        }
    } sc[4];
    bool staged = false;
    uint32_t last_set = 0;
    const BatchClass &last_cls() const { return cls[staged ? 0u : plan.back().cls]; }
    DevBuf<double> d_probs_dbg;
    DevBuf<uint16_t> d_counts_dbg;
    DevBuf<unsigned long long> d_sub_alloc;
    struct ResultSet {
        DevBuf<uint8_t> d_status;
        DevBuf<uint32_t> d_t_all, d_nrows_all, d_n_rows, d_flags, d_ndist;
        DevBuf<double> d_gs, d_z;
        DevBuf<unsigned long long> d_hq, d_row_start, d_cursor;
        DevBuf<DevRow> d_arena;
        uint64_t arena_cap = 0;
        uint64_t side_base = 0;
        PinBuf<unsigned long long> h_side_base;
        DevBuf<uint32_t> d_fin_t, d_fin_row_count, d_fin_lineage, d_fin_node, d_fin_depth;
        DevBuf<uint8_t> d_fin_status, d_fin_depth8, d_fin_hund;
        DevBuf<double> d_fin_gs, d_fin_local, d_fin_conf;
        DevBuf<unsigned long long> d_fin_row_begin, d_fin_cursor;
        uint64_t fin_cap = 0;
        DevBuf<uint32_t> d_perm, d_iperm;
        DevBuf<uint32_t> d_exact_grp;
        DevBuf<uint32_t> d_peak2, d_peak, d_sel_t, d_sel_row_count;
        DevBuf<uint8_t> d_strand, d_sel_status;
        DevBuf<double> d_sel_gs;
        DevBuf<unsigned long long> d_sel_row_begin;
        hipEvent_t ev_select = nullptr;
        DevBuf<uint32_t> d_nearest2, d_ties2, d_nearest, d_ties;
        bool has_nearest = false;
        uint64_t n_user = 0;
        bool has_peak = false;
        hipEvent_t ev_exact = nullptr;
        PinBuf<uint32_t> h_flags;
        hipEvent_t ev_flags = nullptr;
        std::vector<hipEvent_t> ev_sub;
        PinBuf<unsigned long long> h_cursor_sub, h_fin_sub;
        uint64_t n_q = 0;
        uint32_t n_sub = 0, n_side = 0;
        uint32_t in_set = 0;
        bool dev_exact = false;
        bool stream_dl = false;
        bool profiled = false;
        struct Bytes { uint64_t order, groups, rest; };
        Bytes bytes() const {
            return {(d_perm.n + d_iperm.n) * 4, d_exact_grp.n * 4,
                    d_status.n + (d_t_all.n + d_nrows_all.n + d_n_rows.n + d_ndist.n) * 4 + (d_gs.n + d_z.n + d_hq.n + d_row_start.n) * 8 + d_arena.n * sizeof(DevRow) +
                        (d_fin_t.n + d_fin_row_count.n + d_fin_lineage.n + d_fin_node.n + d_fin_depth.n) * 4 + d_fin_status.n + d_fin_depth8.n + d_fin_hund.n +
                        (d_fin_gs.n + d_fin_local.n + d_fin_conf.n + d_fin_row_begin.n) * 8};
        }
        void destroy_events() {
            for (auto e : ev_sub) (void)hipEventDestroy(e);
            if (ev_exact) (void)hipEventDestroy(ev_exact);
            if (ev_flags) (void)hipEventDestroy(ev_flags);
            if (ev_select) (void)hipEventDestroy(ev_select);
        }
    } rs[2];
    uint32_t rs_w = 0;
    ResultSet &res() { return rs[rs_w]; }
    std::vector<hipEvent_t> events;
    uint32_t n_sub_last = 0;
    std::vector<hipEvent_t> ev_near;
    uint32_t n_near_last = 0;
    struct HostRes {
        PinBuf<uint32_t> v_row_lineage, v_row_node, v_row_depth;
        PinBuf<uint8_t> v_row_depth8, v_row_hund;
        PinBuf<uint32_t> h_t;
        PinBuf<uint8_t> h_status;
        PinBuf<double> v_row_conf, v_row_local;
        PinBuf<double> h_gs;
        PinBuf<unsigned long long> v_row_begin;
        PinBuf<uint32_t> v_row_count;
        PinBuf<uint8_t> h_strand;
        PinBuf<uint32_t> h_peak;
        PinBuf<uint32_t> h_nearest, h_ties;
        bool has_nearest = false;
// ... 68 lines not shown
int bind(rtx_index *ix);
int ensure_events(rtx_index *ix, size_t count);

struct SubBatch {
    uint32_t sb, nq, set;
    uint64_t q0;
    const rtx_index::BatchClass *cls;
    hipStream_t s;
    bool timed;
    bool timed_all;
};
SubBatch sub_batch_of(rtx_index *ix, uint32_t sb, bool timed);
uint8_t *counts_lo(rtx_index *ix, rtx_index::Scratch &sc);
uint16_t *counts_hi(rtx_index *ix, const rtx_index::BatchClass &k, rtx_index::Scratch &sc);
uint32_t counts_rows_layout(const rtx_index *ix, const rtx_index::BatchClass &k);
uint32_t diet_rows(const rtx_index *ix, uint32_t B);
int ensure_full_counts(rtx_index *ix, const rtx_index::BatchClass &k, rtx_index::Scratch &sc);
hipEvent_t stage_event(rtx_index *ix, const SubBatch &b, int stage, int which);
int enqueue_kmer(rtx_index *ix, const SubBatch &b, hipStream_t s);
int enqueue_hit(rtx_index *ix, const SubBatch &b, uint32_t flags, hipStream_t s, int part = 0, hipStream_t s_mid = nullptr);
int enqueue_count(rtx_index *ix, const SubBatch &b, uint32_t flags, hipStream_t s_mid = nullptr);
int enqueue_prob_prefix(rtx_index *ix, const SubBatch &b, bool fuse_walk, bool prob_only = false);
int enqueue_walk(rtx_index *ix, const SubBatch &b, const double *prefix, hipStream_t s);
int order_batch(rtx_index *ix, bool cluster);
void record_batch(rtx_index *ix);
int begin_run(rtx_index *ix, uint32_t *n_sub_out, bool *timed_out, bool cluster);
int enqueue_batch(rtx_index *ix, uint32_t flags);
int ensure_prob_tables(rtx_index *ix, uint32_t tmax, bool *usable);
uint32_t length_class(uint64_t len);
uint64_t class3_max_len();
int prepare_workspace(rtx_index *ix, uint64_t n_queries, const uint64_t cls_n[5], const uint64_t cls_max[5]);
int prepare_workspace_single(rtx_index *ix, uint64_t n_queries, uint64_t tmax, uint64_t max_len);
int plan_sub_batches(rtx_index *ix);
int alloc_scratch_set(rtx_index *ix, uint32_t k);
constexpr uint32_t kSideSet = 3;
int node_tables(rtx_index *ix);
int alloc_result_set(rtx_index *ix, rtx_index::ResultSet &r, uint64_t n_queries, uint64_t min_arena = 0);
int settle_join(rtx_index *ix);
int alloc_final(rtx_index *ix, rtx_index::ResultSet &r, uint64_t n_queries);
int enqueue_finalise(rtx_index *ix, const SubBatch &b, hipStream_t s);
int enqueue_profile(rtx_index *ix, rtx_index::ResultSet &r);
void set_derep_hash_mask(uint64_t mask);
int enqueue_text(rtx_index *ix, const rtx_index::ResultSet &r);


struct ItemList {
    size_t np, ntiles;
    ItemList(size_t nq, size_t tiles) : np((nq + 1u) / 2u), ntiles(tiles) {}
    size_t cap() const { return np * ntiles; }
    size_t end() const { return cap() + 9u; }
    uint32_t *items(uint32_t *p) const { return p; }
    uint32_t *count(uint32_t *p) const { return p + cap(); }
};
struct ItemsLayout : ItemList {
    using ItemList::ItemList;
    size_t total() const { return end() + 2u * np; }
    uint32_t *pair_live(uint32_t *p) const { return p + end(); }
    uint32_t *offsets(uint32_t *p) const { return p + end() + np; }
};
struct FineItemsLayout : ItemList {
    using ItemList::ItemList;
    size_t total() const { return end() + ntiles; }
    uint32_t *cursors(uint32_t *p) const { return p + end(); }
};
struct HeavyItemsLayout : ItemList {
    using ItemList::ItemList;
    size_t total() const { return end(); }
};
struct LiveLayout {
    uint32_t ntiles;
    uint32_t words() const { return (ntiles + 31u) / 32u + 1u; }
    size_t total(size_t B) const { return (B + 1u) * words(); }
};

inline size_t counts_elems(const rtx_index *ix, int planes, size_t rows) { return ix->packs(planes) ? rows * ix->npad * 5 / 8 : rows * ix->npad; }

struct ScratchNeed {
    size_t kmers = 0, rows = 0, dmask = 0, counts = 0, hist = 0 , prefix = 0, urec = 0;
    size_t prob_scratch = 0;
    size_t nsparse = 0, srows = 0, t = 0, nrows = 0, order = 0, tilemax = 0, nu = 0;
    size_t tile_ub = 0, best_key = 0, prune_thr = 0, prune_i1 = 0, best = 0, live = 0, items = 0;
    size_t heavy = 0, heavy_items = 0, fine_items = 0;
    size_t rec_nslots = 0, rec_slots = 0, rec_cnt = 0, rec = 0, cnt_row = 0, cnt_cursor = 0;
    ScratchNeed &set_queries(const rtx_index *ix, size_t B) {
        const size_t nt = ix->ntiles;
        t = nrows = order = best_key = prune_thr = prune_i1 = rec_nslots = cnt_row = B;
        nsparse = tilemax = tile_ub = B * nt;
        srows = B * nt * (kSegMaxSparseRows + 1);
        nu = (B + 1u) / 2u;
        best = B * kPruneBestWords;
        live = LiveLayout{ix->ntiles}.total(B);
        items = ItemsLayout(B, nt).total();
        heavy = B + 1u;
        heavy_items = HeavyItemsLayout(B, ix->u_ntiles).total();
        fine_items = FineItemsLayout(B, ix->f_ntiles).total();
        rec_slots = rec_cnt = B * kRecMaxSlots;
        rec = B * ix->rec_slots() * ix->rec_seg_len;
        cnt_cursor = 4;
        return *this;
    }
    void add_class(const rtx_index *ix, const rtx_index::BatchClass &kc, size_t B, size_t cnt_rows) {
        auto up = [](size_t &a, size_t v) { a = std::max(a, v); };
        up(kmers, B * kc.kstride);
        up(rows, B * kc.rstride);
        up(dmask, B * ix->ntiles * (kc.rstride / 64));
        up(counts, counts_elems(ix, kc.planes, cnt_rows));
        up(prefix, cnt_rows * ix->n_bnd_local);
        up(hist, B * kc.hstride);
        up(urec, ((B + 1u) / 2u) * 2u * kc.rstride);
        if (kc.huge) up(prob_scratch, B * ((prob_table_lds_bytes(kc.tmax) + 7) / 8));
    }
};

inline ScratchNeed scratch_set_need(const rtx_index *ix, uint32_t k) {
    ScratchNeed n;
    size_t b_max = 1;
    for (uint32_t c = 0; c < ix->n_cls; c++) {
        const rtx_index::BatchClass &kc = ix->cls[c];
        if (kc.side != (k == kSideSet)) continue;
        const size_t B = kc.sub_batch;
        b_max = std::max(b_max, B);
        const bool diet = kc.will_prune && ix->rec_opt != 0u && ix->n_refs == ix->n_total && ix->n_bnd_local == ix->n_bnd;
        n.add_class(ix, kc, B, diet ? diet_rows(ix, (uint32_t)B) : B);
    }
    return n.set_queries(ix, b_max);
}

inline uint64_t class_per_q(const rtx_index *ix, const rtx_index::BatchClass &k) {
    return (uint64_t)k.kstride * 2 + (uint64_t)k.rstride * 12 + 4 + (uint64_t)ix->ntiles * (k.rstride / 8 + ((kSegMaxSparseRows + 1) * 4 + 10)) + (ix->packs(k.planes) ? ix->npad * 5 / 4 : ix->npad * 2) +
           (uint64_t)k.hstride * 12 + (uint64_t)ix->n_bnd_local * 8 + 64 + (k.huge ? prob_table_lds_bytes(k.tmax) : 0) +
           (k.will_prune ? (uint64_t)ix->ntiles * 2 + 12 + (ix->ntiles + 31u) / 32u * 2u + 2u + kPruneBestWords * 4 +
                               ((uint64_t)ix->ntiles + 2u) * 2u   +
                               (ix->d_fbitmap.p ? (uint64_t)ix->f_ntiles * 2u + 1u : 0u)  +
                               (ix->rec_opt && ix->n_refs == ix->n_total ? (uint64_t)std::min<uint32_t>(ix->rec_opt, kRecMaxSlots) * 32768u + kRecMaxSlots * 6u + 2u : 0u)
                           : 0);
}

}
```

raxtax_amd/csrc/rtx_kernels.hpp:

```cpp
#pragma once

#include <hip/hip_runtime.h>

#include <cstdint>

#include "raxtax_hip.h"
#include "rtx_math.hpp"

namespace rtx {

#ifndef RTX_NODE_TYPES_DEFINED
#define RTX_NODE_TYPES_DEFINED
enum NodeType : uint8_t { kInner = 0, kTaxon = 1, kSequence = 2 };
#endif

constexpr uint32_t kWalkMaxRows = 208;
constexpr uint32_t kSegSlotEntries = 16, kSegSparseMax = 16, kSegMaxSparseRows = 255;
constexpr uint32_t kSegPad = 8192;
__host__ __device__ inline uint32_t seg_pad(uint32_t i) { return kSegPad + ((i & 63u) << 2); }
constexpr uint32_t kKmerFewLive = 8;
constexpr uint32_t kHitListCap = 1024;

struct DevRow {
    uint32_t node;
// ... 169 lines not shown
    uint32_t *flags_out;
};

struct HitParams {
    const uint32_t *bitmap;
    uint32_t n_rows1;
    uint32_t stride_bytes;
    uint64_t n_refs;
    uint32_t ref_base;
    const uint32_t *rows;
    uint32_t rstride;
    const unsigned long long *dmask;
    const uint32_t *nrows;
    uint32_t zero_row;
    uint32_t lds_cnt8_off;
    const uint32_t *srows;
    const uint32_t *nsparse;
    const uint16_t *segslots;
    uint32_t ntiles;
    const uint32_t *t;
    uint16_t *counts;
    uint8_t *counts_lo;
    uint16_t *counts_hi;
    uint64_t npad;
    uint32_t *hist;
    uint32_t hstride;
    uint16_t *tile_max;
    uint32_t flags;
    uint64_t q0;
    const uint32_t *perm;
    ExactRef exact;
    uint32_t nq;
    uint32_t *group_rows;
    uint32_t group_base;
    const uint2 *pair_urec;
    const uint32_t *pair_nu;
    uint32_t pair_ustride;
    const uint32_t *live;
    uint32_t live_words;
    const uint16_t *prune_thr;
    const uint32_t *items;
    uint32_t *n_items;
    uint16_t *bounds_tile_ub;
    uint32_t bounds_tile_stride, bounds_ntiles;
    uint32_t *bounds_best;
    const uint8_t *bounds_heavy;
    uint64_t fine_n_refs;
    uint32_t fine_ref_ntiles;
    unsigned long long *fine_stats;
    RecordRef rec;
    const uint32_t *cnt_row;
};
struct Bounds2Params {
    const uint32_t *abitmap;
    const uint8_t *bbitmap;
    uint32_t n_rows1, n_atiles, ntiles, zero_row;
    const uint2 *pair_urec;
    const uint32_t *pair_nu;
    uint32_t pair_ustride, nq;
    const uint32_t *t;
    uint16_t *tile_ub;
    uint32_t tile_ub_stride;
    uint32_t *best_key;
    uint32_t delta_ct, delta_cm, delta_lo, delta_hi;
    uint8_t *heavy;
    uint32_t heavy_max;
    uint32_t *group_rows;
    uint32_t group_base;
};
struct HitParams;
void launch_bounds2(hipStream_t s, const Bounds2Params &p, uint32_t nq, int planes, const HitParams &hp, uint32_t u_ntiles, uint32_t *items);
constexpr uint32_t kTwoLevelMinTiles = 16;
void launch_bounds2_build(hipStream_t s, const uint32_t *ubitmap, uint32_t n_rows1, uint32_t u_ntiles, uint8_t *bbitmap, uint32_t *abitmap);
constexpr uint32_t kFineShift = 3;
constexpr uint32_t kFineMinLive = 4;
constexpr uint32_t kFineMinTiles = 16;

constexpr uint32_t kPruneStatCopies = 64;
#ifndef RTX_PRUNE_SHIFT
#define RTX_PRUNE_SHIFT 6
#endif
constexpr uint32_t kPruneShift = RTX_PRUNE_SHIFT;
static_assert(kPruneShift >= 3 && kPruneShift <= 6, "blocks of 8 .. 64 references");
constexpr uint32_t kPruneBestWords = 66;
struct PruneParams {
    const uint16_t *tile_ub;
    const uint32_t *best_key;
    uint32_t tile_ub_stride, ntiles, nq;
    uint64_t n_refs;
    uint64_t n_total;
    uint32_t ref_base;
    uint32_t phase;
    uint32_t *best;
    const uint2 *cbitmap;
    const uint32_t *bitmap;
    uint32_t n_rows1, stride_bytes;
    const uint32_t *rows;
    uint32_t rstride;
    const uint32_t *nrows, *t;
    uint32_t flags;
    uint64_t q0;
    const uint32_t *perm;
    ExactRef exact;
    const double *lnfact, *inv;
    uint32_t nlf;
    uint32_t *hist;
    uint32_t hstride;
    uint32_t *live;
    uint32_t live_words;
    uint32_t *pair_live;
    uint16_t *thr_out;
    uint16_t *i1_out;
    unsigned long long *stats;
    uint32_t *detail;
    RecordRef rec;
    uint32_t rec_max_slots;
    uint32_t *cnt_row;
    uint32_t *cnt_cursor;
    uint32_t cnt_cap;
    uint32_t *flags_out;
};
constexpr uint32_t kPruneDetailWords = 72;
struct ProbTables;
void launch_prune(hipStream_t s, const PruneParams &p, const ProbTables &tb, uint32_t nq);
void launch_block_major_build(hipStream_t s, const uint32_t *bitmap, uint32_t n_rows1, uint32_t ntiles, uint32_t stride_bytes, uint8_t *cbitmap);

struct ProbTables {
    double *cmf;
    double *ratio;
    const uint64_t *off;
    const uint32_t *moff;
    uint16_t *ilo;
    uint16_t *sat;
    uint32_t tmax;
};


struct ProbParams {
    const uint32_t *order;
    const uint32_t *t;
    const uint32_t *hist;
    uint32_t hstride;
    uint32_t tmax;
    uint32_t n1max;
    const double *lnfact;
    uint64_t n_refs;
    uint64_t q0;
    double *table_z;
    double *z;
    double *gs;
    uint8_t *status;
    uint32_t *ndist;
    const uint16_t *prune_thr;
    const uint16_t *prune_i1;
    double *gscratch;
    uint32_t gstride;
};

constexpr uint32_t kWalkSubAllocs = 128;
constexpr uint32_t kWalkSubStride = 16;
constexpr uint32_t kWalkSubMinQueries = 4096;
constexpr uint32_t kWalkChunkRows = 64;
struct WalkParams {
    const uint8_t *status;
    uint64_t q0;
    const double *prefix;
    uint32_t n_bnd;
    const uint4 *rec;
    DevRow *arena;
    unsigned long long arena_cap;
    unsigned long long *arena_cursor;
    unsigned long long *sub_alloc;
    uint32_t *n_rows;
    unsigned long long *row_start;
    uint32_t *flags_out;
};

struct FinaliseParams {
    const uint8_t *status;
    const uint32_t *t_all;
    const double *gs;
    const uint32_t *n_rows;
    const unsigned long long *row_start;
    const DevRow *arena;
    unsigned long long arena_cap;
    const uint32_t *perm;
    uint64_t q0;
    uint32_t nq;
    const uint8_t *node_depth, *node_sig0;
    const uint32_t *node_begin;
    const double *node_eb;
    uint32_t D;
    uint32_t *o_t;
    uint8_t *o_status;
    double *o_gs;
    unsigned long long *o_row_begin;
    uint32_t *o_row_count;
    uint32_t *r_lineage, *r_node, *r_depth;
    uint8_t *r_depth8, *r_hund;
    double *r_local, *r_conf;
    unsigned long long row_cap;
    unsigned long long *fin_cursor;
    uint32_t *flags_out;
};

constexpr int kBounds2MaxPlanes = 11;

struct PrefixParams {
    const uint8_t *status;
    const uint32_t *t;
    uint32_t tz_in_lds;
    uint64_t q0;
    const uint16_t *counts;
    const uint8_t *counts_lo;
    const uint16_t *counts_hi;
    uint32_t packed;
    uint64_t npad;
    const double *table_z;
    uint32_t hstride;
    uint64_t n_refs;
    const uint8_t *bnd_bits;
    const uint32_t *bnd_rank;
    double *prefix;
    uint32_t n_bnd;
    const uint16_t *tile_max;
    uint32_t ntiles;
    const uint16_t *prune_thr;
    unsigned long long *prune_stats;
    uint32_t fuse_walk;
    WalkParams walk;
    const uint16_t *rec_nslots;
    const uint32_t *cnt_row;
};


struct TailParams {
    RecordRef rec;
    const uint32_t *t;
    const double *table_z;
    uint32_t hstride;
    const uint8_t *bnd_bits;
    const uint32_t *bnd_rank;
    double *prefix;
    uint32_t *cnt_cursor;
    uint32_t cnt_cap;
    uint32_t *flags_out;
    uint32_t n_bnd;
    uint32_t nq;
    WalkParams walk;
    unsigned long long *prefix_stats;
    unsigned long long *stats;
};
void launch_records_tail(hipStream_t s, const TailParams &p, uint32_t nq);

void launch_bitmap_build(hipStream_t s, const uint64_t *off, const uint32_t *post, const uint32_t *row_of,
                         uint32_t *bitmap, uint32_t stride_words, uint32_t n_rows1, uint32_t ref_lo, uint32_t ref_hi, uint32_t shift = 0);
void launch_ref_kmer_mark(hipStream_t s, const uint8_t *bases, const uint64_t *off, uint64_t n_refs, uint32_t *present);
void launch_ref_bitmap_set(hipStream_t s, const uint8_t *bases, const uint64_t *off, uint64_t n_refs,
                           const uint32_t *row_of, uint32_t *bitmap, uint32_t stride_words, uint32_t n_rows1, uint32_t shift = 0);
void launch_row_len_pack(hipStream_t s, const uint32_t *row_of, const uint32_t *list_len, uint2 *out);
void launch_row_popcount(hipStream_t s, const uint32_t *row_of, const uint32_t *bitmap, uint32_t stride_words, uint32_t n_rows1,
                         uint32_t *list_len);
void launch_kmer_extract(hipStream_t s, const KmerParams &p, uint32_t nq);
void launch_hit_count(hipStream_t s, const HitParams &p, uint32_t nq, uint32_t ntiles, int planes);
void launch_pair_union(hipStream_t s, const uint32_t *rows, const uint32_t *nrows, uint32_t rstride, uint32_t nq, uint2 *urec,
                       uint32_t *nu, uint32_t ustride);
void launch_hit_count_pair(hipStream_t s, const HitParams &p, uint32_t nq, uint32_t ntiles, int planes);
void launch_live_items(hipStream_t s, const uint32_t *live, uint32_t live_words, const uint32_t *pair_live, uint32_t nq, uint32_t ntiles, uint32_t *off,
                       uint32_t *items, uint32_t *n_items);
void launch_hit_count_pair_bounds(hipStream_t s, const HitParams &p, uint32_t nq, uint32_t u_ntiles, int planes);
void launch_hit_count_pair_bounds_items(hipStream_t s, const HitParams &p, uint32_t nq, uint32_t u_ntiles, int planes);
void launch_fine_bounds(hipStream_t s, const HitParams &p, uint32_t nq, uint32_t ntiles, uint32_t f_ntiles, uint32_t *pair_live, uint32_t *cnt,
                        uint32_t *items, uint32_t *n_items, int planes);
size_t prob_table_lds_bytes(uint32_t tmax);
void launch_prob_table(hipStream_t s, const ProbParams &p, uint32_t nq);
size_t prob_lookup_lds_bytes(uint32_t tmax);
void launch_prob_tables_build(hipStream_t s, const ProbTables &tb, const double *lf, const double *inv);
void launch_prob_order(hipStream_t s, const uint32_t *t, uint32_t nq, uint32_t *order);
void launch_prob_lookup(hipStream_t s, const ProbParams &p, const ProbTables &tb, uint32_t nq);
void launch_seg_popcount(hipStream_t s, const uint32_t *bitmap, uint32_t stride_bytes, uint32_t n_rows1, uint32_t ntiles, uint16_t *pop);
void launch_seg_emit(hipStream_t s, const uint32_t *bitmap, uint32_t stride_bytes, uint32_t n_rows1, uint32_t ntiles,
                     const uint32_t *seginfo, uint32_t seg_stride, uint16_t *slots);
void launch_sketch(hipStream_t s, const uint8_t *bases, const uint64_t *off, uint32_t n_q, uint64_t *keys, uint32_t *idx);
void launch_invert_perm(hipStream_t s, const uint32_t *perm, uint32_t n, uint32_t *inv);
constexpr uint32_t kLocTableEntries = 1u << 24;
void launch_loc_mark(hipStream_t s, const uint8_t *bases, const uint64_t *off, uint64_t n_refs, uint32_t *pos_min, uint32_t *cnt);
void launch_loc_finish(hipStream_t s, uint32_t *pos_min, const uint32_t *cnt);
void launch_locator(hipStream_t s, const uint8_t *bases, const uint64_t *off, uint32_t n_q, const uint32_t *table, uint64_t n_refs,
                    uint64_t *keys);
void launch_identity_perm(hipStream_t s, uint32_t n, uint32_t *perm, uint32_t *inv);
int cluster_sort(hipStream_t s, void *tmp, size_t *tmp_bytes, const uint64_t *keys_in, uint64_t *keys_out, const uint32_t *idx_in,
                 uint32_t *perm_out, size_t n, bool with_class = false);
void launch_class_keys(hipStream_t s, uint64_t *keys, const uint64_t *off, uint32_t n, const uint64_t lim[4], bool from_index, uint32_t *idx);
void launch_taxon_prefix(hipStream_t s, const PrefixParams &p, uint32_t nq);
void launch_lineage_walk(hipStream_t s, const WalkParams &p, uint32_t nq);
void launch_finalise(hipStream_t s, const FinaliseParams &p);
void launch_probs_expand(hipStream_t s, const uint16_t *counts, const double *tz, uint64_t n, double *out);
void launch_rehist(hipStream_t s, const uint16_t *counts, uint64_t npad, uint64_t n_refs, const uint32_t *t, uint32_t *hist,
                   uint32_t hstride, uint16_t *tile_max, uint32_t ntiles, uint32_t nq);
void launch_counts_unpack(hipStream_t s, const uint8_t *lo, const uint16_t *hi, uint64_t n, uint16_t *out);

}
```

raxtax_amd/csrc/rtx_prob_tables.hip:

```cpp
#include <hip/hip_runtime.h>

#include "rtx_kernels.hpp"
#include "rtx_math.hpp"
#include "rtx_wave.hpp"

namespace rtx {

__global__ __launch_bounds__(256) void prob_tables_build_kernel(ProbTables tb, const double *__restrict__ lf,
                                                                const double *__restrict__ inv) {
    const uint32_t t = blockIdx.y + 2;
    const uint32_t m = blockIdx.x * blockDim.x + threadIdx.x;
    if (t > tb.tmax || m >= t) return;
    const uint32_t n = t >> 1, n1 = n + 1;
    double *C = tb.cmf + tb.off[t] + (size_t)m * n1;
    double *R = tb.ratio + tb.off[t] + (size_t)m * n1;
    uint16_t *meta_ilo = tb.ilo + tb.moff[t];
    uint16_t *meta_sat = tb.sat + tb.moff[t];
    if (m == 0) {
        for (uint32_t i = 0; i <= n; i++) { C[i] = 0.0; R[i] = i == 0 ? 1.0 : 0.0; }
        meta_ilo[0] = 0;
        meta_sat[0] = 1;
        return;
    }
    const double ln_total = ln_binom_tab(lf, t + n - 1, n);
    PmfState st = pmf_start(lf, t, n, m, ln_total);
    uint32_t sat = n + 1, ilo = n;
    bool ilo_found = false;
    for (uint32_t i = 0; i <= n; i++) {
        if (i > 0) {
            const double c_old = st.c;
            const int k_old = st.k;
            pmf_step(st, inv, t, n, m, i);
            if (sat == n + 1 && st.c == c_old && k_old == 0 && st.k == 0) sat = i;
        }
        const bool live = st.k == 0 && st.c > 0.0;
        C[i] = live ? log(st.c) : -INFINITY;
        R[i] = live ? st.v / st.c : 0.0;
        if (!ilo_found && ln_pmf_tab(lf, t, n, m, i, ln_total) >= kLnNegligibleP) { ilo = i; ilo_found = true; }
    }
    meta_ilo[m] = (uint16_t)ilo;
    meta_sat[m] = (uint16_t)sat;
}

typedef uint32_t u32x2_t __attribute__((ext_vector_type(2)));
__device__ __forceinline__ double row_load_f64(const double *table, uint32_t off, uint32_t end, uint32_t voff) {
    const __amdgpu_buffer_rsrc_t rsrc = __builtin_amdgcn_make_buffer_rsrc(const_cast<double *>(table), 0, end, 0x00027000);
    const u32x2_t v = __builtin_amdgcn_raw_buffer_load_b64(rsrc, voff, off, 0);
    return __hiloint2double((int)v.y, (int)v.x);
}

#ifndef RTX_PROB_WAVES
#define RTX_PROB_WAVES 6
#endif
__global__ __launch_bounds__(256, RTX_PROB_WAVES) void prob_lookup_kernel(ProbParams p, ProbTables tb) {
    extern __shared__ double smem[];
    __shared__ uint32_t s_D, s_nact;
    __shared__ uint32_t s_nlive[16];
    const uint32_t q = p.order ? p.order[blockIdx.x] : blockIdx.x;
    const uint32_t tid = threadIdx.x, lane = tid & 63u, wave = tid >> 6;
    const uint64_t gq = p.q0 + q;
    const uint32_t t = p.t[q];
    const uint32_t n = t >> 1;
    const uint32_t n1 = n + 1;
    double *Pi = smem;
    double *red = Pi + p.n1max;
    double *Ppart = red + 16;
    double *tzl = Ppart + 64;
    uint32_t *row_h = reinterpret_cast<uint32_t *>(tzl + (p.tmax + 2));
    uint16_t *row_m = reinterpret_cast<uint16_t *>(row_h + (p.tmax + 18));
    uint16_t *row_sat = row_m + (p.tmax + 18);
    uint16_t *ms = row_sat + (p.tmax + 18);
    uint32_t *hl = reinterpret_cast<uint32_t *>(ms + ((p.tmax + 18 + 1) & ~1u));
    uint32_t *row_off = hl + (p.tmax + 4);
    uint32_t *row_end = row_off + (p.tmax + 18);
    const uint32_t *hist = p.hist + (size_t)q * p.hstride;
    double *tz = p.table_z + (size_t)q * p.hstride;
    const double *lf = p.lnfact;

    {
        const uint32_t hlim = p.hstride < p.tmax + 4u ? p.hstride : p.tmax + 4u;
        for (uint32_t m = tid; m < hlim; m += 256) hl[m] = hist[m];
    }
    if (t == 0) {
        if (tid == 0) { p.status[gq] = RTX_Q_NO_KMERS; p.z[gq] = 0.0; p.gs[gq] = 0.0; p.ndist[gq] = 0; }
        return;
    }
    __syncthreads();
    const uint32_t u_thr = p.prune_thr ? p.prune_thr[q] : 0u;
    if (u_thr) {
        uint32_t low = 0;
        for (uint32_t m = 1u + tid; m <= u_thr && m <= t; m += 256) {
            low += hl[m];
            hl[m] = 0;
            tz[m] = 0.0;
        }
        if (low) atomicAdd(&hl[0], low);
        __syncthreads();
    }
    if (wave == 0) {
        uint32_t D = 0;
        for (uint32_t m0 = 0; m0 <= t; m0 += 64) {
            const uint32_t m = m0 + lane;
            const bool has = m <= t && hl[m] != 0;
            const unsigned long long bal = __ballot(has);
            if (has) ms[D + __popcll(bal & ((1ull << lane) - 1ull))] = (uint16_t)m;
            D += (uint32_t)__popcll(bal);
        }
        if (lane == 0) { s_D = D; p.ndist[gq] = D; }
    }
    __syncthreads();
    const uint32_t D = s_D;
    const uint32_t M = ms[D - 1];
    const double ln_total = ln_binom_tab(lf, t + n - 1, n);
    if (M == t) {
        for (uint32_t j = tid; j < D; j += 256) {
            const uint32_t m = ms[j];
            tzl[m] = only_last_pmf_tab(lf, t, n, m, ln_total);
        }
    } else {
        if (n == 0) {
            if (tid == 0) { p.status[gq] = RTX_Q_NO_KMERS; p.z[gq] = 0.0; p.gs[gq] = 0.0; }
            return;
        }
        const uint16_t *t_ilo = tb.ilo + tb.moff[t];
        const uint16_t *t_sat = tb.sat + tb.moff[t];
        const double *Ct = tb.cmf + tb.off[t];
        const double *Rt = tb.ratio + tb.off[t];
        uint32_t i_lo = M > 0 ? t_ilo[M] : 0u;
        if (u_thr && p.prune_i1) { const uint32_t i1 = p.prune_i1[q]; i_lo = i1 > i_lo && i1 <= n ? i1 : i_lo; }
        for (uint32_t j = tid; j < D; j += 256) {
            const uint32_t m = ms[D - 1 - j];
            row_h[j] = m ? t_sat[m] : 0u;
        }
        __syncthreads();
        if (wave == 0) {
            uint32_t na = 0;
            if (lane < 16) s_nlive[lane] = 0;
            for (uint32_t j0 = 0; j0 < D; j0 += 64) {
                const uint32_t j = j0 + lane;
                uint32_t m = 0, sat = 0;
                if (j < D) {
                    m = ms[D - 1 - j];
                    sat = row_h[j];
                    if (m && sat <= i_lo) tzl[m] = 0.0;
                }
                const bool keep = m != 0 && sat > i_lo;
                const unsigned long long bal = __ballot(keep);
                if (keep) {
                    const uint32_t pos = na + (uint32_t)__popcll(bal & ((1ull << lane) - 1ull));
                    row_m[pos] = (uint16_t)m;
                    row_sat[pos] = (uint16_t)sat;
                    row_h[pos] = hl[m];
                    row_off[pos] = m * n1 * 8u;
                    row_end[pos] = (m * n1 + (sat < n1 ? sat : n1)) * 8u;
                    const uint32_t nsl = ((sat < n1 ? sat : n1) - i_lo + 63u) >> 6;
                    atomicMax(&s_nlive[(nsl < 16u ? nsl : 16u) - 1u], pos + 1u);
                }
                na += (uint32_t)__popcll(bal);
            }
            const uint32_t padded = (na + 15u) & ~15u;
            if (na + lane < padded) { row_m[na + lane] = 0; row_sat[na + lane] = 0; row_h[na + lane] = 0; row_off[na + lane] = 0; row_end[na + lane] = 0; }
            if (lane == 0) {
                s_nact = na;
                for (int sl = 14; sl >= 0; sl--) s_nlive[sl] = max(s_nlive[sl], s_nlive[sl + 1]);
            }
        }
        __syncthreads();
        const uint32_t nact = s_nact;
        auto slice_sum = [&](uint32_t sl, uint32_t rbeg, uint32_t rstep) -> double {
            const uint32_t voff = (i_lo + sl * 64u + lane) * 8u;
            const uint32_t rend = s_nlive[sl];
            double S = 0.0;
            for (uint32_t r0 = rbeg; r0 < rend; r0 += rstep) {
                const uint32_t l16 = r0 + (lane & 15u);
                const uint32_t ov = row_off[l16], ev = row_end[l16], hv = row_h[l16];
                double c[16];
#pragma unroll
                for (int k = 0; k < 16; k++)
                    c[k] = row_load_f64(Ct, (uint32_t)__builtin_amdgcn_readlane((int)ov, k), (uint32_t)__builtin_amdgcn_readlane((int)ev, k), voff);
#pragma unroll
                for (int k = 0; k < 16; k++) {
                    const uint32_t h = (uint32_t)__builtin_amdgcn_readlane((int)hv, k);
                    S = fma((double)h, c[k], S);
                }
            }
            return S;
        };
        const uint32_t nslices = ((n - i_lo) >> 6) + 1u;
        double S0 = 0.0;
        if (wave < 2) {
            S0 = slice_sum(0, wave * 16u, 32u);
            if (wave == 1) Ppart[lane] = S0;
        } else {
            for (uint32_t sl = wave - 1u; sl < nslices; sl += 2) {
                const double S = slice_sum(sl, 0, 16u);
                const uint32_t i = i_lo + sl * 64u + lane;
                if (i <= n) Pi[i - i_lo] = exp(S);
            }
        }
        __syncthreads();
        if (wave == 0) {
            const uint32_t i = i_lo + lane;
            if (i <= n) Pi[i - i_lo] = exp(S0 + Ppart[lane]);
        }
        __syncthreads();
        for (uint32_t r0 = wave * 8; r0 < nact; r0 += 32) {
            double acc[8];
            uint32_t off[8], end[8];
            uint32_t lmax = 0;
#pragma unroll
            for (int k = 0; k < 8; k++) {
                acc[k] = 0.0;
// ... 101 lines not shown
```

raxtax_amd/csrc/rtx_prune.hip:

```cpp
#include <hip/hip_runtime.h>

#include "rtx_kernels.hpp"
#include "rtx_math.hpp"
#include "rtx_wave.hpp"

namespace rtx {

static constexpr double kPruneLnEps = kPruneLnEpsHD;
static constexpr double kPruneHalfEps = kPruneHalfEpsHD;
#ifndef RTX_PRUNE_WAVES
#define RTX_PRUNE_WAVES 4
#endif
#ifndef RTX_PRUNE_TURNS
#define RTX_PRUNE_TURNS 16
#endif
static constexpr uint32_t kPruneWavesPerBlock = 4;

__device__ __forceinline__ uint32_t wave_max_u32p(uint32_t v) { return wave_max_u32(v); }

__global__ __launch_bounds__(64 * kPruneWavesPerBlock, RTX_PRUNE_WAVES) void prune_kernel(PruneParams p, ProbTables tb) {
    extern __shared__ double prune_lds[];
    for (uint32_t i = threadIdx.x; i < p.nlf; i += 64u * kPruneWavesPerBlock) prune_lds[i] = p.lnfact[i];
    __syncthreads();
    const uint32_t lane = threadIdx.x & 63u, pair = blockIdx.x * kPruneWavesPerBlock + (threadIdx.x >> 6);
// ... 253 lines not shown
                        double lnG = 0.0;
                        unsigned long long hb = __ballot(hm != 0u);
                        const uint32_t iwc = vi ? iw : n;
                        while (hb) {
                            double v[4];
#pragma unroll
                            for (int k = 0; k < 4; k++) {
                                v[k] = 0.0;
                                if (hb) {
                                    const int h = __builtin_ctzll(hb);
                                    hb &= hb - 1ull;
                                    const uint32_t m = (uint32_t)__builtin_amdgcn_readlane((int)hm, h);
                                    v[k] = Ct[(size_t)m * (n + 1) + iwc];
                                }
                            }
#pragma unroll
                            for (int k = 0; k < 4; k++) lnG += v[k];
                        }
                        const double gw = vi && !tail_pt ? exp(lnG) : 0.0;
                        const double ww = vi && !tail_pt ? exp(fmin(0.0, ln_kept + lnG)) : 0.0;
                        const double incl = wave_incl_scan_f64_dpp(ww);
                        const double a_tot = readlane_f64(incl, 63);
                        const double len_tail = vi ? (double)(n - iw + 1u) : 0.0;
                        const double WA = tail_pt ? len_tail * (a_tot + 1.0) : (vi ? incl - ww : 0.0);
                        const double WB = tail_pt ? len_tail : gw;
                        const double nn = (double)p.n_total;
                        const bool has_tail = i1 + 63u <= n;
                        auto sums_at = [&](uint32_t m, double &a, double &b) {
                            const double P = vi && m != 0u ? exp(ln_pmf_tab(lf, t, n, m, iw, ln_total)) : 0.0;
                            a = wave_sum_f64_dpp(P * WA);
                            b = wave_sum_f64_dpp(P * WB);
                        };
                        double gsa = 0.0, gsb = 0.0, far_a = 0.0, far_b = 0.0, n_far = 0.0, mid_a = 0.0, mid_b = 0.0, n_mid = 0.0;
                        bool near = false;
                        if (tile_aware) {
                            const uint32_t m_far = u_max > kPruneFarGap ? u_max - kPruneFarGap : 0u;
                            near = gnd > 0.0 && gub > u_max;
                            const bool mid = gnd > 0.0 && gub > m_far && gub <= u_max;
                            unsigned long long nb = __ballot(near);
                            if ((uint32_t)__popcll(nb) > kPruneMaxNear) {
                                near = gnd > 0.0;
                                const uint32_t gcap = gub < h_min ? gub : h_min - 1u;
                                prune_window_sums(lf, p.inv, t, n, gcap, i1, ln_total, [&](uint32_t l) { return readlane_f64(WA, (int)l); },
                                                  [&](uint32_t l) { return readlane_f64(WB, (int)l); }, gsa, gsb);
                            } else {
                                n_far = wave_sum_f64_dpp(near || mid ? 0.0 : gnd);
                                n_mid = wave_sum_f64_dpp(mid ? gnd : 0.0);
                                if (m_far) sums_at(m_far, far_a, far_b);
                                if (n_mid > 0.0) sums_at(u_max, mid_a, mid_b);
                                while (nb) {
                                    const int g = __builtin_ctzll(nb);
                                    nb &= nb - 1ull;
                                    const uint32_t m = (uint32_t)__builtin_amdgcn_readlane((int)gub, g);
                                    double a, b;
                                    sums_at(m < h_min ? m : h_min - 1u, a, b);
                                    if ((int)lane == g) { gsa = a; gsb = b; }
                                }
                            }
                        }
                        auto crit = [&](uint32_t u) -> bool {
                            bool falling = true;
                            if (has_tail) {
                                const uint32_t j = i1 + 63u;
                                falling = (double)(u + j) * (double)(n - j) < (double)(j + 1u) * (double)(t - u + n - j - 1u);
                            }
                            double a, b;
                            sums_at(u, a, b);
                            if (!tile_aware) return falling && nn * a <= kPruneHalfEps && nn * b <= kPruneHalfEps;
                            const bool dead = gub <= u;
                            return falling && wave_sum_f64_dpp(near ? gnd * (dead ? gsa : a) : 0.0) + n_far * far_a + n_mid * mid_a <= kPruneHalfEps &&
                                   wave_sum_f64_dpp(near ? gnd * (dead ? gsb : b) : 0.0) + n_far * far_b + n_mid * mid_b <= kPruneHalfEps;
                        };
                        uint32_t lo = u_max, hi = h_min - 1u;
                        while (lo < hi) {
                            const uint32_t mid = (lo + hi + 1u) >> 1;
                            if (crit(mid)) lo = mid; else hi = mid - 1u;
                        }
                        u_max = lo;
                    }
                }
            }
        }
        thr[x] = u_max;
        if (lane == 0) { p.thr_out[q] = (uint16_t)u_max; p.i1_out[q] = (uint16_t)(u_max ? i1_q : 0u); }
        if (p.detail && lane == 0) {
            uint32_t *d = p.detail + (size_t)q * kPruneDetailWords;
            d[0] = bb; d[1] = M; d[2] = u_max; d[3] = u_max ? i1_q : 0u; d[4] = ub_best; d[5] = t; d[6] = 0u; d[7] = 0u;
        }
        st[2] += M; st[3] += u_max; st[4] += ub_best; st[5] += 1ull;
        if (ub_best < M) st[6] += 1ull;
    }
    if (p.phase == 1u) return;
    __builtin_amdgcn_fence(__ATOMIC_ACQ_REL, "wavefront");
    __builtin_amdgcn_wave_barrier();
    unsigned long long dead_refs[2] = {0, 0};
    uint32_t n_live = 0, n_qlive = 0;
    uint32_t n_rec[2] = {0u, 0u};
    for (uint32_t T0 = 0; T0 < p.ntiles; T0 += 64) {
        const uint32_t T = T0 + lane;
        bool la = false, lb = false;
        if (T < p.ntiles) {
            la = thr[0] == 0u || (uint32_t)ub_lds[T] > thr[0];
            lb = has_b && (thr[1] == 0u || (uint32_t)ub_lds[p.ntiles + T] > thr[1]);
        }
        const unsigned long long ba = __ballot(la), bb2 = __ballot(lb);
        if (lane == 0) {
            uint32_t *wa = p.live + (size_t)(pair * 2u) * p.live_words, *wb = wa + p.live_words;
            wa[T0 >> 5] = (uint32_t)ba;
            if ((T0 >> 5) + 1u < p.live_words) wa[(T0 >> 5) + 1u] = (uint32_t)(ba >> 32);
            if (has_b) {
                wb[T0 >> 5] = (uint32_t)bb2;
                if ((T0 >> 5) + 1u < p.live_words) wb[(T0 >> 5) + 1u] = (uint32_t)(bb2 >> 32);
            }
        }
        if (T < p.ntiles) {
            const uint64_t lo = (uint64_t)T * 8192u, hi = lo + 8192u < p.n_refs ? lo + 8192u : p.n_refs;
            if (!la) dead_refs[0] += hi - lo;
            if (!lb) dead_refs[1] += hi - lo;
        }
        if (p.rec.nslots) {
            const unsigned long long lt = (1ull << lane) - 1ull;
            const uint32_t ka = n_rec[0] + (uint32_t)__popcll(ba & lt), kb = n_rec[1] + (uint32_t)__popcll(bb2 & lt);
            if (la && ka < kRecMaxSlots) p.rec.slots[(size_t)(pair * 2u) * kRecMaxSlots + ka] = (uint16_t)T;
            if (lb && kb < kRecMaxSlots) p.rec.slots[(size_t)(pair * 2u + 1u) * kRecMaxSlots + kb] = (uint16_t)T;
            n_rec[0] += (uint32_t)__popcll(ba);
            n_rec[1] += (uint32_t)__popcll(bb2);
        }
        n_live += (uint32_t)__popcll(ba | bb2);
        n_qlive += (uint32_t)__popcll(ba) + (uint32_t)__popcll(bb2);
    }
    if (p.rec.nslots) {
        const uint32_t cap = p.rec_max_slots < kRecMaxSlots ? p.rec_max_slots : kRecMaxSlots;
        const bool ra = thr[0] != 0u && n_rec[0] != 0u && n_rec[0] <= cap, rb = has_b && thr[1] != 0u && n_rec[1] != 0u && n_rec[1] <= cap;
        if (lane < kRecMaxSlots) {
            p.rec.cnt[(size_t)(pair * 2u) * kRecMaxSlots + lane] = 0u;
            if (has_b) p.rec.cnt[(size_t)(pair * 2u + 1u) * kRecMaxSlots + lane] = 0u;
        }
        if (lane == 0) {
            p.rec.nslots[pair * 2u] = (uint16_t)(ra ? n_rec[0] : 0u);
            if (has_b) p.rec.nslots[pair * 2u + 1u] = (uint16_t)(rb ? n_rec[1] : 0u);
            if (p.cnt_row) {
                auto row_for = [&](bool records) -> uint32_t {
                    if (records) return 0xFFFFFFFFu;
                    const uint32_t r = atomicAdd(p.cnt_cursor, 1u);
                    if (r < p.cnt_cap) return r;
                    atomicOr(p.flags_out, 4u);
                    return 0xFFFFFFFFu;
                };
                p.cnt_row[pair * 2u] = row_for(ra);
                if (has_b) p.cnt_row[pair * 2u + 1u] = row_for(rb);
            }
        }
    }
#pragma unroll
    for (int d = 32; d >= 1; d >>= 1) { dead_refs[0] += __shfl_xor(dead_refs[0], d, 64); dead_refs[1] += __shfl_xor(dead_refs[1], d, 64); }
    if (lane == 0) {
        p.hist[(size_t)(pair * 2u) * p.hstride] = (uint32_t)dead_refs[0];
        if (has_b) p.hist[(size_t)(pair * 2u + 1u) * p.hstride] = (uint32_t)dead_refs[1];
    }
    if (lane == 0 && p.pair_live) p.pair_live[pair] = n_live;
    st[7] = n_qlive;
    if (p.stats) {
        st[0] = n_live; st[1] = 1ull;
        unsigned long long mine = 0;
#pragma unroll
        for (int k = 0; k < 8; k++) mine = lane == (uint32_t)k ? st[k] : mine;
        if (lane < 8u && mine) atomicAdd(&p.stats[(size_t)(pair & (kPruneStatCopies - 1u)) * 8u + lane], mine);
    }
}

__global__ __launch_bounds__(256) void block_major_build_kernel(const uint32_t *__restrict__ bitmap, uint32_t n_rows1, uint32_t stride_bytes,
                                                                uint8_t *__restrict__ cbitmap) {
    const uint32_t row = blockIdx.x, tile = blockIdx.y, word = threadIdx.x;
    const uint32_t v = bitmap[((size_t)tile * n_rows1 + row) * 256u + word];
    if (v == 0u) return;
    const uint32_t l = word >> 2, wi = word & 3u, L = tile_lanes(stride_bytes, tile);
    if (l >= L) return;
#pragma unroll
    for (uint32_t k = 0; k < 4u; k++) {
        const uint32_t byte = (v >> (8u * k)) & 0xFFu;
        if (byte == 0u) continue;
        const uint32_t ref0 = tile * 8192u + ((wi * 4u + k) * L + l) * 8u;
        cbitmap[((size_t)(ref0 >> 6) * n_rows1 + row) * 8u + ((ref0 & 63u) >> 3)] = (uint8_t)byte;
    }
}
void launch_block_major_build(hipStream_t s, const uint32_t *bitmap, uint32_t n_rows1, uint32_t ntiles, uint32_t stride_bytes, uint8_t *cbitmap) {
    hipLaunchKernelGGL(block_major_build_kernel, dim3(n_rows1, ntiles), dim3(256), 0, s, bitmap, n_rows1, stride_bytes, cbitmap);
}

void launch_prune(hipStream_t s, const PruneParams &p, const ProbTables &tb, uint32_t nq) {
    const uint32_t pairs = (nq + 1u) / 2u;
    hipLaunchKernelGGL(prune_kernel, dim3((pairs + kPruneWavesPerBlock - 1u) / kPruneWavesPerBlock), dim3(64 * kPruneWavesPerBlock),
                       (size_t)p.nlf * sizeof(double) + (size_t)kPruneWavesPerBlock * 2 * p.ntiles * sizeof(uint16_t), s, p, tb);
}

}
```

raxtax_amd/csrc/rtx_records.hip:

```cpp
#include <hip/hip_runtime.h>

#include "rtx_kernels.hpp"
#include "rtx_walk.hpp"
#include "rtx_wave.hpp"

namespace rtx {

constexpr uint32_t kTailEntries = 256;

struct EntryPrefix {
    const uint32_t *f;
    const double *S;
    uint32_t n;
    __device__ __forceinline__ double operator()(uint32_t b) const {
        uint32_t lo = 0;
#pragma unroll
        for (uint32_t step = kTailEntries; step >= 1u; step >>= 1) {
            const uint32_t probe = lo + step;
            const bool ok = probe <= n && f[probe <= n ? probe - 1u : 0u] <= b;
            lo = ok ? probe : lo;
        }
        return lo ? S[lo - 1u] : 0.0;
    }
};

__global__ __launch_bounds__(64) void records_tail_kernel(TailParams p) {
    extern __shared__ double tail_lds[];
    const uint32_t q = blockIdx.x, lane = threadIdx.x;
    const uint32_t ns = p.rec.nslots[q];
    if (ns == 0u) return;
    const uint64_t gq = p.walk.q0 + q;
    if (p.walk.status[gq] != RTX_Q_OK) {
        if (lane == 0) { p.walk.n_rows[gq] = 0; p.walk.row_start[gq] = 0; }
        return;
    }
    WalkLds &L = *reinterpret_cast<WalkLds *>(tail_lds);
    double *ent_S = reinterpret_cast<double *>(reinterpret_cast<char *>(tail_lds) + ((sizeof(WalkLds) + 15u) & ~(size_t)15u));
    uint32_t *ent_f = reinterpret_cast<uint32_t *>(ent_S + kTailEntries);
    const double *__restrict__ tz = p.table_z + (size_t)q * p.hstride;
    const uint32_t tq = p.t[q];
    const uint32_t tile_v = lane < ns ? (uint32_t)p.rec.slots[(size_t)q * kRecMaxSlots + lane] : 0u;
    const uint32_t cnt_v = lane < ns ? p.rec.cnt[(size_t)q * kRecMaxSlots + lane] : 0u;
    const unsigned long long lt_mask = (1ull << lane) - 1ull;
    double *__restrict__ Prow = p.prefix + (size_t)q * p.n_bnd;
    uint32_t E = 0, n_rec = 0;
    bool slow = false;
    for (uint32_t pass = 0; pass < 2u; pass++) {
        double carry = 0.0;
        uint32_t filled = 0;
        E = 0;
        n_rec = 0;
        for (uint32_t k = 0; k < ns; k++) {
            const uint32_t tile = (uint32_t)__builtin_amdgcn_readlane((int)tile_v, (int)k);
            uint32_t c = (uint32_t)__builtin_amdgcn_readlane((int)cnt_v, (int)k);
            c = c < p.rec.seg_len ? c : p.rec.seg_len;
            const uint32_t *seg = p.rec.rec + ((size_t)q * p.rec.stride + k) * p.rec.seg_len;
            n_rec += c;
            for (uint32_t i0 = 0; i0 < c; i0 += 64) {
                const uint32_t i = i0 + lane;
                const bool valid = i < c;
                const uint32_t r = seg[valid ? i : 0u];
                const uint32_t ref = tile * 8192u + (r & 8191u);
                uint32_t cnt = r >> 13;
                cnt = cnt <= tq ? cnt : tq;
                const uint32_t ch = ref >> 3, j = ref & 7u;
                const double tv = tz[cnt];
                const uint32_t rk = p.bnd_rank[ch], bits = p.bnd_bits[ch];
                const double pv = valid ? tv : 0.0;
                const uint32_t f = valid ? rk + (uint32_t)__popc(bits & ((1u << j) - 1u)) : 0xFFFFFFFFu;
                const double incl = carry + wave_incl_scan_f64_dpp(pv);
                const uint32_t f_next = (uint32_t)__shfl_down((int)f, 1, 64);
                const bool is_end = valid && (lane == 63u || f_next != f);
                const unsigned long long em = __ballot(is_end);
                if (pass == 0u) {
                    const uint32_t pos = E + (uint32_t)__popcll(em & lt_mask);
                    if (is_end && pos < kTailEntries) { ent_f[pos] = f; ent_S[pos] = incl; }
                } else {
                    const uint32_t f_first = (uint32_t)__builtin_amdgcn_readfirstlane((int)f);
                    for (uint32_t b = filled + lane; b < f_first; b += 64) Prow[b] = carry;
                    unsigned long long rest = em;
                    while (rest) {
                        const int e = __builtin_ctzll(rest);
                        rest &= rest - 1ull;
                        const uint32_t fa = (uint32_t)__builtin_amdgcn_readlane((int)f, e);
                        const double sa = readlane_f64(incl, e);
                        if (rest) {
                            const uint32_t fb = (uint32_t)__builtin_amdgcn_readlane((int)f_next, e);
                            for (uint32_t b = fa + lane; b < fb; b += 64) Prow[b] = sa;
                            filled = fb;
                        } else {
                            if (lane == 0) Prow[fa] = sa;
                            filled = fa;
                        }
                    }
                }
                E += (uint32_t)__popcll(em);
                carry = readlane_f64(incl, 63);
            }
        }
        if (pass == 0u) {
            if (E <= kTailEntries) break;
            slow = true;
            if (p.cnt_cursor) {
                uint32_t r = 0;
                if (lane == 0) r = atomicAdd(p.cnt_cursor, 1u);
                r = (uint32_t)__builtin_amdgcn_readfirstlane((int)r);
                if (r >= p.cnt_cap) {
                    if (lane == 0) { atomicOr(p.flags_out, 4u); p.walk.n_rows[gq] = 0; p.walk.row_start[gq] = 0; }
                    return;
                }
                Prow = p.prefix + (size_t)r * p.n_bnd;
            }
        } else {
            for (uint32_t b = filled + lane; b < p.n_bnd; b += 64) Prow[b] = carry;
        }
    }
    if (p.prefix_stats) {
        const uint32_t need = (uint32_t)__popcll(__ballot(lane < ns && cnt_v != 0u));
        if (lane < 2u) atomicAdd(&p.prefix_stats[(size_t)(q & (kPruneStatCopies - 1u)) * 8u + lane], lane == 0u ? (unsigned long long)need : 1ull);
    }
    if (p.stats && lane < 4u) {
        const unsigned long long v = lane == 0u ? n_rec : (lane == 1u ? 1u : (lane == 2u ? E : (slow ? 1u : 0u)));
        if (v) atomicAdd(&p.stats[(size_t)(q & (kPruneStatCopies - 1u)) * 8u + lane], v);
    }
    wave_lds_sync();
    if (!slow) {
        lineage_walk_wave(p.walk, q, lane, L, EntryPrefix{ent_f, ent_S, E});
    } else {
        __builtin_amdgcn_fence(__ATOMIC_RELEASE, "workgroup");
        __builtin_amdgcn_fence(__ATOMIC_ACQUIRE, "workgroup");
        lineage_walk_wave(p.walk, q, lane, L, GapPrefix{Prow, nullptr});
    }
}

void launch_records_tail(hipStream_t s, const TailParams &p, uint32_t nq) {
    const size_t lds = ((sizeof(WalkLds) + 15u) & ~(size_t)15u) + (size_t)kTailEntries * 12u;
    hipLaunchKernelGGL(records_tail_kernel, dim3(nq), dim3(64), lds, s, p);
}

}
```

raxtax_amd/csrc/rtx_wave.hpp:

```cpp
#pragma once

#include <hip/hip_runtime.h>

#include <cstdint>

namespace rtx {

__device__ __forceinline__ uint32_t lane_id() { return threadIdx.x & 63u; }

__device__ __forceinline__ uint32_t wave_incl_scan_u32(uint32_t v) {
    v += (uint32_t)__builtin_amdgcn_update_dpp(0, (int)v, 0x111, 0xF, 0xF, true);
    v += (uint32_t)__builtin_amdgcn_update_dpp(0, (int)v, 0x112, 0xF, 0xF, true);
    v += (uint32_t)__builtin_amdgcn_update_dpp(0, (int)v, 0x114, 0xF, 0xF, true);
    v += (uint32_t)__builtin_amdgcn_update_dpp(0, (int)v, 0x118, 0xF, 0xF, true);
    const uint32_t r0 = (uint32_t)__builtin_amdgcn_readlane((int)v, 15), r1 = (uint32_t)__builtin_amdgcn_readlane((int)v, 31),
                   r2 = (uint32_t)__builtin_amdgcn_readlane((int)v, 47);
    const uint32_t row = lane_id() >> 4;
    return v + (row == 0 ? 0u : (row == 1 ? r0 : (row == 2 ? r0 + r1 : r0 + r1 + r2)));
}

__device__ __forceinline__ uint32_t row16_max_u32(uint32_t v) {
    uint32_t o;
    o = (uint32_t)__builtin_amdgcn_update_dpp(0, (int)v, 0xB1, 0xF, 0xF, true); v = o > v ? o : v;
    o = (uint32_t)__builtin_amdgcn_update_dpp(0, (int)v, 0x4E, 0xF, 0xF, true); v = o > v ? o : v;
    o = (uint32_t)__builtin_amdgcn_update_dpp(0, (int)v, 0x141, 0xF, 0xF, true); v = o > v ? o : v;
    o = (uint32_t)__builtin_amdgcn_update_dpp(0, (int)v, 0x140, 0xF, 0xF, true); v = o > v ? o : v;
    return v;
}

__device__ __forceinline__ uint32_t wave_max_u32(uint32_t v) {
    v = row16_max_u32(v);
    const uint32_t a = (uint32_t)__builtin_amdgcn_readlane((int)v, 0), b = (uint32_t)__builtin_amdgcn_readlane((int)v, 16),
                   c = (uint32_t)__builtin_amdgcn_readlane((int)v, 32), d = (uint32_t)__builtin_amdgcn_readlane((int)v, 48);
    const uint32_t ab = a > b ? a : b, cd = c > d ? c : d;
    return ab > cd ? ab : cd;
}

__device__ __forceinline__ double wave_sum_f64(double v) {
#pragma unroll
    for (int d = 32; d >= 1; d >>= 1) v += __shfl_xor(v, d, 64);
    return v;
}

__device__ __forceinline__ double dpp_mov_f64(double v, int ctrl_sel) {
    int lo = __double2loint(v), hi = __double2hiint(v);
    switch (ctrl_sel) {
        case 0: lo = __builtin_amdgcn_update_dpp(0, lo, 0xB1, 0xF, 0xF, true); hi = __builtin_amdgcn_update_dpp(0, hi, 0xB1, 0xF, 0xF, true); break;
        case 1: lo = __builtin_amdgcn_update_dpp(0, lo, 0x4E, 0xF, 0xF, true); hi = __builtin_amdgcn_update_dpp(0, hi, 0x4E, 0xF, 0xF, true); break;
        case 2: lo = __builtin_amdgcn_update_dpp(0, lo, 0x141, 0xF, 0xF, true); hi = __builtin_amdgcn_update_dpp(0, hi, 0x141, 0xF, 0xF, true); break;
        case 3: lo = __builtin_amdgcn_update_dpp(0, lo, 0x140, 0xF, 0xF, true); hi = __builtin_amdgcn_update_dpp(0, hi, 0x140, 0xF, 0xF, true); break;
        default: lo = __builtin_amdgcn_update_dpp(0, lo, 0x128, 0xF, 0xF, true); hi = __builtin_amdgcn_update_dpp(0, hi, 0x128, 0xF, 0xF, true); break;
    }
    return __hiloint2double(hi, lo);
}
__device__ __forceinline__ double readlane_f64(double v, int l) {
    return __hiloint2double(__builtin_amdgcn_readlane(__double2hiint(v), l), __builtin_amdgcn_readlane(__double2loint(v), l));
}
__device__ __forceinline__ double wave_sum_f64_dpp(double v) {
    v += dpp_mov_f64(v, 0);
    v += dpp_mov_f64(v, 1);
    v += dpp_mov_f64(v, 2);
    v += dpp_mov_f64(v, 3);
    return (readlane_f64(v, 0) + readlane_f64(v, 16)) + (readlane_f64(v, 32) + readlane_f64(v, 48));
}

__device__ __forceinline__ double wave_sum8_f64(const double (&a)[8]) {
    const uint32_t lane = lane_id();
    const bool b2 = lane & 4u, b1 = lane & 2u, b0 = lane & 1u;
    double b[4], c[2];
#pragma unroll
    for (int j = 0; j < 4; j++) b[j] = (b2 ? a[j + 4] : a[j]) + dpp_mov_f64(b2 ? a[j] : a[j + 4], 2);
#pragma unroll
    for (int j = 0; j < 2; j++) c[j] = (b1 ? b[j + 2] : b[j]) + dpp_mov_f64(b1 ? b[j] : b[j + 2], 1);
    double d = (b0 ? c[1] : c[0]) + dpp_mov_f64(b0 ? c[0] : c[1], 0);
    d += dpp_mov_f64(d, 4);
    d += __shfl_xor(d, 16, 64);
    d += __shfl_xor(d, 32, 64);
    return d;
}

__device__ __forceinline__ double wave_prod_f64_dpp(double v) {
    v *= dpp_mov_f64(v, 0);
    v *= dpp_mov_f64(v, 1);
    v *= dpp_mov_f64(v, 2);
    v *= dpp_mov_f64(v, 3);
    return (readlane_f64(v, 0) * readlane_f64(v, 16)) * (readlane_f64(v, 32) * readlane_f64(v, 48));
}

__device__ __forceinline__ double dpp_shr_f64(double v, int n) {
    int lo = __double2loint(v), hi = __double2hiint(v);
    switch (n) {
// ... 30 lines not shown
```

Baseline: 13.06 million.

## Pack per-query head into 32-byte record and software-pipeline records tail loads

The prune kernel now writes a 32-byte per-query header holding t, prune threshold, i1, record slot count and the table offsets. The prob lookup and records tail kernels read it with two vector loads instead of several scattered scalar and dependent table loads. The records tail kernel also issues its early loads up front, flattens the nested slot loop into one loop that prefetches the next chunk, and the prob kernel skips histogram entries below the prune threshold. The cost is extra scratch memory and more complex control flow, plus a risk of mismatch if the header and the separate arrays fall out of sync.

After: 13.14 million, median of 6. About the same (+0.7%).

```diff
diff --git a/include/raxtax_hip.h b/include/raxtax_hip.h
--- a/include/raxtax_hip.h
+++ b/include/raxtax_hip.h
@@ -103,6 +103,7 @@
 uint64_t rtx_index_device_bytes(const rtx_index *index);
 uint64_t rtx_index_workspace_bytes(const rtx_index *index);
 int rtx_index_workspace_parts(const rtx_index *index, uint64_t out[9]);
+int rtx_query_head_layout(uint32_t out[8]);
 int rtx_index_set_batch(rtx_index *index, uint32_t sub_batch);
 #define RTX_OPT_SUB_BATCH 1
 #define RTX_OPT_PROB_MODE 2
diff --git a/raxtax_amd/_lib.py b/raxtax_amd/_lib.py
--- a/raxtax_amd/_lib.py
+++ b/raxtax_amd/_lib.py
@@ -109,6 +109,7 @@
     "rtx_index_device_bytes": (C.c_uint64, [C.c_void_p]),
     "rtx_index_workspace_bytes": (C.c_uint64, [C.c_void_p]),
     "rtx_index_workspace_parts": (C.c_int, [C.c_void_p, u64p]),
+    "rtx_query_head_layout": (C.c_int, [u32p]),
     "rtx_index_set_batch": (C.c_int, [C.c_void_p, C.c_uint32]),
     "rtx_set_default_option": (C.c_int, [C.c_int, C.c_uint64]),
     "rtx_index_set_option": (C.c_int, [C.c_void_p, C.c_int, C.c_uint64]),
diff --git a/raxtax_amd/api.py b/raxtax_amd/api.py
--- a/raxtax_amd/api.py
+++ b/raxtax_amd/api.py
@@ -233,6 +233,10 @@
     check(lib.rtx_profile_format(*args, buf, n))
     return buf.raw[:n].decode()
 
+
+QUERY_HEAD = np.dtype({"names": ["t", "u_thr", "i1", "nslots", "off", "moff", "pad"],
+                       "formats": [np.uint32, np.uint32, np.uint32, np.uint32, np.uint64, np.uint32, np.uint32],
+                       "offsets": [0, 4, 8, 12, 16, 24, 28], "itemsize": 32})
 
 DEFAULT_SEGMENT_CLASSES = 1
 
@@ -335,6 +339,10 @@
     def workspace_bytes(self) -> int:
         return self._lib.rtx_index_workspace_bytes(self._h)
 
+    @staticmethod
+    def query_head_bytes(sub_batch: int, scratch_sets: int = 1) -> int:
+        return int(sub_batch) * int(scratch_sets) * QUERY_HEAD.itemsize
+
     def workspace_parts(self) -> dict:
         out = np.zeros(9, dtype=np.uint64)
         check(self._lib.rtx_index_workspace_parts(self._h, ptr(out, u64p)))
diff --git a/raxtax_amd/csrc/rtx_api_batch.hip b/raxtax_amd/csrc/rtx_api_batch.hip
--- a/raxtax_amd/csrc/rtx_api_batch.hip
+++ b/raxtax_amd/csrc/rtx_api_batch.hip
@@ -250,6 +250,7 @@
     pr.i1_out = sc.d_prune_i1.p;
     pr.stats = ix->d_prune_stats.p;
     pr.detail = ix->debug_taps && ix->d_prune_detail.n >= (size_t)b.nq * kPruneDetailWords ? ix->d_prune_detail.p : nullptr;
+    pr.head = part == 0 && k.use_tables && sc.d_qhead.n >= b.nq ? sc.d_qhead.p : nullptr;
     return pr;
 }
 
@@ -279,6 +280,7 @@
     rtx_index::ResultSet &r = ix->res();
     const rtx_index::BatchClass &k = *b.cls;
     ix->last_set = b.set;
+    sc.head_on = false;
     HitParams hp = hit_params(ix, b, flags);
     const bool prune = run_prunes(ix, k);
     if (k.pair && part != 2) {
@@ -322,6 +324,7 @@
             hp.cnt_row = sc.d_cnt_row.p;
         }
         launch_prune(s, pr, prob_tables(ix), b.nq);
+        sc.head_on = pr.head != nullptr;
         if (part == 1) { RTX_HIP(hipGetLastError()); return RTX_OK; }
         if (part == 0 && ix->fine_opt && ix->d_fbitmap.p && k.pair && sc.d_fine_items.p) {
             const FineItemsLayout fine(b.nq, ix->f_ntiles);
@@ -391,6 +394,7 @@
     if (k.use_tables) {
         launch_prob_order(s, sc.d_t.p, b.nq, sc.d_order.p);
         pp.order = sc.d_order.p;
+        pp.head = pp.prune_thr && sc.head_on ? sc.d_qhead.p : nullptr;
         launch_prob_lookup(s, pp, prob_tables(ix), b.nq);
     } else {
         if (k.huge) {
@@ -439,6 +443,7 @@
         TailParams tp{};
         tp.rec = record_ref(ix, sc, r);
         tp.t = sc.d_t.p;
+        tp.head = pp.head;
         tp.table_z = sc.d_table_z.p;
         tp.hstride = k.hstride;
         tp.bnd_bits = ix->d_bnd_bits.p;
@@ -1141,6 +1146,7 @@
                 sc.d_rec.alloc(n.rec) || sc.d_cnt_row.alloc(n.cnt_row) || sc.d_cnt_cursor.alloc(n.cnt_cursor))
                 sc.d_rec.release();
         }
+        if (ix->n_refs == ix->n_total && sc.d_qhead.alloc(n.qhead)) sc.d_qhead.release();
     }
     return RTX_OK;
 }
diff --git a/raxtax_amd/csrc/rtx_api_index.hip b/raxtax_amd/csrc/rtx_api_index.hip
--- a/raxtax_amd/csrc/rtx_api_index.hip
+++ b/raxtax_amd/csrc/rtx_api_index.hip
@@ -702,6 +702,13 @@
     out[5] = all > named ? all - named : 0;
     return RTX_OK;
 }
+int rtx_query_head_layout(uint32_t out[8]) {
+    if (!out) { set_error("null argument"); return RTX_ERR_INVALID; }
+    const uint32_t v[8] = {(uint32_t)sizeof(QueryHead), (uint32_t)alignof(QueryHead), (uint32_t)offsetof(QueryHead, t), (uint32_t)offsetof(QueryHead, u_thr),
+                           (uint32_t)offsetof(QueryHead, i1), (uint32_t)offsetof(QueryHead, nslots), (uint32_t)offsetof(QueryHead, off), (uint32_t)offsetof(QueryHead, moff)};
+    for (int i = 0; i < 8; i++) out[i] = v[i];
+    return RTX_OK;
+}
 int rtx_index_set_batch(rtx_index *index, uint32_t sub_batch) {
     if (!index) { set_error("null index handle"); return RTX_ERR_INVALID; }
     index->uploaded = index->ran = index->synced = false;
diff --git a/raxtax_amd/csrc/rtx_index.hpp b/raxtax_amd/csrc/rtx_index.hpp
--- a/raxtax_amd/csrc/rtx_index.hpp
+++ b/raxtax_amd/csrc/rtx_index.hpp
@@ -280,12 +280,14 @@
         DevBuf<uint16_t> d_rec_nslots, d_rec_slots;
         DevBuf<uint32_t> d_rec_cnt, d_rec;
         DevBuf<uint32_t> d_cnt_row, d_cnt_cursor;
+        DevBuf<QueryHead> d_qhead;
+        bool head_on = false;
         template <class S, class F>
         static void each(S &s, F &&f) {
             f(s.d_kmers); f(s.d_counts); f(s.d_tilemax); f(s.d_rows); f(s.d_t); f(s.d_nrows); f(s.d_hist); f(s.d_order); f(s.d_srows); f(s.d_nsparse);
             f(s.d_dmask); f(s.d_table_z); f(s.d_prefix); f(s.d_urec); f(s.d_nu); f(s.d_live); f(s.d_best_key); f(s.d_items); f(s.d_tile_ub); f(s.d_prune_thr);
             f(s.d_prune_i1); f(s.d_best); f(s.d_heavy); f(s.d_heavy_items); f(s.d_fine_items); f(s.d_rec_nslots); f(s.d_rec_slots); f(s.d_rec_cnt); f(s.d_rec);
-            f(s.d_cnt_row); f(s.d_cnt_cursor);
+            f(s.d_cnt_row); f(s.d_cnt_cursor); f(s.d_qhead);
         }
         void release_all() { each(*this, [](auto &b) { b.release(); }); }
         uint64_t bytes() const {
@@ -520,9 +522,10 @@
     size_t tile_ub = 0, best_key = 0, prune_thr = 0, prune_i1 = 0, best = 0, live = 0, items = 0;
     size_t heavy = 0, heavy_items = 0, fine_items = 0;
     size_t rec_nslots = 0, rec_slots = 0, rec_cnt = 0, rec = 0, cnt_row = 0, cnt_cursor = 0;
+    size_t qhead = 0;
     ScratchNeed &set_queries(const rtx_index *ix, size_t B) {
         const size_t nt = ix->ntiles;
-        t = nrows = order = best_key = prune_thr = prune_i1 = rec_nslots = cnt_row = B;
+        t = nrows = order = best_key = prune_thr = prune_i1 = rec_nslots = cnt_row = qhead = B;
         nsparse = tilemax = tile_ub = B * nt;
         srows = B * nt * (kSegMaxSparseRows + 1);
         nu = (B + 1u) / 2u;
diff --git a/raxtax_amd/csrc/rtx_kernels.hpp b/raxtax_amd/csrc/rtx_kernels.hpp
--- a/raxtax_amd/csrc/rtx_kernels.hpp
+++ b/raxtax_amd/csrc/rtx_kernels.hpp
@@ -275,6 +275,16 @@
 #endif
 constexpr uint32_t kPruneShift = RTX_PRUNE_SHIFT;
 static_assert(kPruneShift >= 3 && kPruneShift <= 6, "blocks of 8 .. 64 references");
+struct alignas(32) QueryHead {
+    uint32_t t;
+    uint32_t u_thr;
+    uint32_t i1;
+    uint32_t nslots;
+    uint64_t off;
+    uint32_t moff;
+    uint32_t pad;
+};
+static_assert(sizeof(QueryHead) == 32 && alignof(QueryHead) == 32, "a head is one 32-byte line: two 16-byte loads");
 constexpr uint32_t kPruneBestWords = 66;
 struct PruneParams {
     const uint16_t *tile_ub;
@@ -312,6 +322,7 @@
     uint32_t *cnt_cursor;
     uint32_t cnt_cap;
     uint32_t *flags_out;
+    QueryHead *head;
 };
 constexpr uint32_t kPruneDetailWords = 72;
 struct ProbTables;
@@ -346,6 +357,7 @@
     uint32_t *ndist;
     const uint16_t *prune_thr;
     const uint16_t *prune_i1;
+    const QueryHead *head;
     double *gscratch;
     uint32_t gstride;
 };
@@ -430,6 +442,7 @@
 struct TailParams {
     RecordRef rec;
     const uint32_t *t;
+    const QueryHead *head;
     const double *table_z;
     uint32_t hstride;
     const uint8_t *bnd_bits;
diff --git a/raxtax_amd/csrc/rtx_prob_tables.hip b/raxtax_amd/csrc/rtx_prob_tables.hip
--- a/raxtax_amd/csrc/rtx_prob_tables.hip
+++ b/raxtax_amd/csrc/rtx_prob_tables.hip
@@ -59,9 +59,13 @@
     const uint32_t q = p.order ? p.order[blockIdx.x] : blockIdx.x;
     const uint32_t tid = threadIdx.x, lane = tid & 63u, wave = tid >> 6;
     const uint64_t gq = p.q0 + q;
-    const uint32_t t = p.t[q];
-    const uint32_t n = t >> 1;
-    const uint32_t n1 = n + 1;
+    uint4 h0 = make_uint4(0, 0, 0, 0), h1 = h0;
+    if (p.head) {
+        const uint4 *h = reinterpret_cast<const uint4 *>(p.head + q) + lane_zero();
+        h0 = h[0];
+        h1 = h[1];
+    }
+    const uint32_t t_arr = p.head ? 0u : p.t[q];
     double *Pi = smem;
     double *red = Pi + p.n1max;
     double *Ppart = red + 16;
@@ -81,12 +85,26 @@
         const uint32_t hlim = p.hstride < p.tmax + 4u ? p.hstride : p.tmax + 4u;
         for (uint32_t m = tid; m < hlim; m += 256) hl[m] = hist[m];
     }
+    uint32_t t, u_thr = 0, i1_q = 0, t_moff = 0;
+    uint64_t t_off = 0;
+    if (p.head) {
+        t = (uint32_t)__builtin_amdgcn_readfirstlane((int)h0.x);
+        u_thr = (uint32_t)__builtin_amdgcn_readfirstlane((int)h0.y);
+        i1_q = (uint32_t)__builtin_amdgcn_readfirstlane((int)h0.z);
+        t_off = (uint64_t)(uint32_t)__builtin_amdgcn_readfirstlane((int)h1.x) | (uint64_t)(uint32_t)__builtin_amdgcn_readfirstlane((int)h1.y) << 32;
+        t_moff = (uint32_t)__builtin_amdgcn_readfirstlane((int)h1.z);
+    } else {
+        t = t_arr;
+    }
+    const uint32_t n = t >> 1;
+    const uint32_t n1 = n + 1;
     if (t == 0) {
         if (tid == 0) { p.status[gq] = RTX_Q_NO_KMERS; p.z[gq] = 0.0; p.gs[gq] = 0.0; p.ndist[gq] = 0; }
         return;
     }
-    __syncthreads();
-    const uint32_t u_thr = p.prune_thr ? p.prune_thr[q] : 0u;
+    const double ln_total = ln_binom_tab(lf, t + n - 1, n);
+    __syncthreads();
+    if (!p.head) u_thr = p.prune_thr ? p.prune_thr[q] : 0u;
     if (u_thr) {
         uint32_t low = 0;
         for (uint32_t m = 1u + tid; m <= u_thr && m <= t; m += 256) {
@@ -99,8 +117,9 @@
     }
     if (wave == 0) {
         uint32_t D = 0;
-        for (uint32_t m0 = 0; m0 <= t; m0 += 64) {
-            const uint32_t m = m0 + lane;
+        const uint32_t skip = u_thr < t ? u_thr : t;
+        for (uint32_t m0 = 0; m0 <= t - skip; m0 += 64) {
+            const uint32_t m = m0 + lane ? skip + m0 + lane : 0u;
             const bool has = m <= t && hl[m] != 0;
             const unsigned long long bal = __ballot(has);
             if (has) ms[D + __popcll(bal & ((1ull << lane) - 1ull))] = (uint16_t)m;
@@ -111,7 +130,6 @@
     __syncthreads();
     const uint32_t D = s_D;
     const uint32_t M = ms[D - 1];
-    const double ln_total = ln_binom_tab(lf, t + n - 1, n);
     if (M == t) {
         for (uint32_t j = tid; j < D; j += 256) {
             const uint32_t m = ms[j];
@@ -122,12 +140,13 @@
             if (tid == 0) { p.status[gq] = RTX_Q_NO_KMERS; p.z[gq] = 0.0; p.gs[gq] = 0.0; }
             return;
         }
-        const uint16_t *t_ilo = tb.ilo + tb.moff[t];
-        const uint16_t *t_sat = tb.sat + tb.moff[t];
-        const double *Ct = tb.cmf + tb.off[t];
-        const double *Rt = tb.ratio + tb.off[t];
+        if (!p.head) { t_moff = tb.moff[t]; t_off = tb.off[t]; }
+        const uint16_t *t_ilo = tb.ilo + t_moff;
+        const uint16_t *t_sat = tb.sat + t_moff;
+        const double *Ct = tb.cmf + t_off;
+        const double *Rt = tb.ratio + t_off;
         uint32_t i_lo = M > 0 ? t_ilo[M] : 0u;
-        if (u_thr && p.prune_i1) { const uint32_t i1 = p.prune_i1[q]; i_lo = i1 > i_lo && i1 <= n ? i1 : i_lo; }
+        if (u_thr && (p.head || p.prune_i1)) { const uint32_t i1 = p.head ? i1_q : p.prune_i1[q]; i_lo = i1 > i_lo && i1 <= n ? i1 : i_lo; }
         for (uint32_t j = tid; j < D; j += 256) {
             const uint32_t m = ms[D - 1 - j];
             row_h[j] = m ? t_sat[m] : 0u;
diff --git a/raxtax_amd/csrc/rtx_prune.hip b/raxtax_amd/csrc/rtx_prune.hip
--- a/raxtax_amd/csrc/rtx_prune.hip
+++ b/raxtax_amd/csrc/rtx_prune.hip
@@ -359,6 +359,16 @@
             }
         }
         thr[x] = u_max;
+        if (p.head && lane == 0) {
+            QueryHead *h = p.head + q;
+            const bool tab = t <= tb.tmax;
+            h->t = t;
+            h->u_thr = (uint32_t)(uint16_t)u_max;
+            h->i1 = (uint32_t)(uint16_t)(u_max ? i1_q : 0u);
+            h->off = tab ? tb.off[t] : 0ull;
+            h->moff = tab ? tb.moff[t] : 0u;
+            h->pad = 0u;
+        }
         if (lane == 0) { p.thr_out[q] = (uint16_t)u_max; p.i1_out[q] = (uint16_t)(u_max ? i1_q : 0u); }
         if (p.detail && lane == 0) {
             uint32_t *d = p.detail + (size_t)q * kPruneDetailWords;
@@ -416,6 +426,10 @@
         if (lane == 0) {
             p.rec.nslots[pair * 2u] = (uint16_t)(ra ? n_rec[0] : 0u);
             if (has_b) p.rec.nslots[pair * 2u + 1u] = (uint16_t)(rb ? n_rec[1] : 0u);
+            if (p.head) {
+                p.head[pair * 2u].nslots = (uint16_t)(ra ? n_rec[0] : 0u);
+                if (has_b) p.head[pair * 2u + 1u].nslots = (uint16_t)(rb ? n_rec[1] : 0u);
+            }
             if (p.cnt_row) {
                 auto row_for = [&](bool records) -> uint32_t {
                     if (records) return 0xFFFFFFFFu;
@@ -429,6 +443,10 @@
             }
         }
     }
+    if (p.head && !p.rec.nslots && lane == 0) {
+        p.head[pair * 2u].nslots = 0u;
+        if (has_b) p.head[pair * 2u + 1u].nslots = 0u;
+    }
 #pragma unroll
     for (int d = 32; d >= 1; d >>= 1) { dead_refs[0] += __shfl_xor(dead_refs[0], d, 64); dead_refs[1] += __shfl_xor(dead_refs[1], d, 64); }
     if (lane == 0) {
diff --git a/raxtax_amd/csrc/rtx_records.hip b/raxtax_amd/csrc/rtx_records.hip
--- a/raxtax_amd/csrc/rtx_records.hip
+++ b/raxtax_amd/csrc/rtx_records.hip
@@ -27,10 +27,26 @@
 __global__ __launch_bounds__(64) void records_tail_kernel(TailParams p) {
     extern __shared__ double tail_lds[];
     const uint32_t q = blockIdx.x, lane = threadIdx.x;
-    const uint32_t ns = p.rec.nslots[q];
+    const uint64_t gq = p.walk.q0 + q;
+    uint32_t ns, tq;
+    if (p.head) {
+        const uint4 h0 = *(reinterpret_cast<const uint4 *>(p.head + q) + lane_zero());
+        tq = h0.x;
+        ns = h0.w;
+    } else {
+        ns = p.rec.nslots[q];
+        tq = p.t[q];
+    }
+    const uint32_t status = p.walk.status[gq];
+    const uint32_t lane_s = lane < kRecMaxSlots ? lane : 0u;
+    const uint32_t tile_w = p.rec.slots[(size_t)q * kRecMaxSlots + lane_s], cnt_w = p.rec.cnt[(size_t)q * kRecMaxSlots + lane_s];
+    const uint32_t *const seg_q = p.rec.rec + (size_t)q * p.rec.stride * p.rec.seg_len;
+    const uint32_t r_first = seg_q[lane < p.rec.seg_len ? lane : 0u];
+    asm volatile("" ::"v"(status), "v"(tile_w), "v"(cnt_w), "v"(r_first));
+    ns = (uint32_t)__builtin_amdgcn_readfirstlane((int)ns);
+    tq = (uint32_t)__builtin_amdgcn_readfirstlane((int)tq);
     if (ns == 0u) return;
-    const uint64_t gq = p.walk.q0 + q;
-    if (p.walk.status[gq] != RTX_Q_OK) {
+    if (status != RTX_Q_OK) {
         if (lane == 0) { p.walk.n_rows[gq] = 0; p.walk.row_start[gq] = 0; }
         return;
     }
@@ -38,65 +54,81 @@
     double *ent_S = reinterpret_cast<double *>(reinterpret_cast<char *>(tail_lds) + ((sizeof(WalkLds) + 15u) & ~(size_t)15u));
     uint32_t *ent_f = reinterpret_cast<uint32_t *>(ent_S + kTailEntries);
     const double *__restrict__ tz = p.table_z + (size_t)q * p.hstride;
-    const uint32_t tq = p.t[q];
-    const uint32_t tile_v = lane < ns ? (uint32_t)p.rec.slots[(size_t)q * kRecMaxSlots + lane] : 0u;
-    const uint32_t cnt_v = lane < ns ? p.rec.cnt[(size_t)q * kRecMaxSlots + lane] : 0u;
+    const uint32_t tile_v = lane < ns ? tile_w : 0u;
+    const uint32_t cnt_v = lane < ns ? (cnt_w < p.rec.seg_len ? cnt_w : p.rec.seg_len) : 0u;
+    auto advance = [&](uint32_t &k, uint32_t &i0) {
+        i0 += 64u;
+        if (k < ns && i0 < (uint32_t)__builtin_amdgcn_readlane((int)cnt_v, (int)k)) return;
+        i0 = 0;
+        do k++; while (k < ns && (uint32_t)__builtin_amdgcn_readlane((int)cnt_v, (int)k) == 0u);
+    };
+    auto load_turn = [&](uint32_t k, uint32_t i0) -> uint32_t {
+        const uint32_t c = (uint32_t)__builtin_amdgcn_readlane((int)cnt_v, (int)k);
+        const uint32_t i = i0 + lane;
+        return seg_q[(size_t)(k < ns ? k : 0u) * p.rec.seg_len + (i < c ? i : 0u)];
+    };
+    uint32_t k_first = 0, i_first = 0;
+    if ((uint32_t)__builtin_amdgcn_readlane((int)cnt_v, 0) == 0u) advance(k_first, i_first);
+    const uint32_t r_head = lane < (uint32_t)__builtin_amdgcn_readlane((int)cnt_v, 0) ? r_first : (uint32_t)__builtin_amdgcn_readfirstlane((int)r_first);
     const unsigned long long lt_mask = (1ull << lane) - 1ull;
     double *__restrict__ Prow = p.prefix + (size_t)q * p.n_bnd;
-    uint32_t E = 0, n_rec = 0;
+    uint32_t E = 0;
+    const uint32_t n_rec = (uint32_t)__builtin_amdgcn_readlane((int)wave_incl_scan_u32(cnt_v), 63);
     bool slow = false;
     for (uint32_t pass = 0; pass < 2u; pass++) {
         double carry = 0.0;
         uint32_t filled = 0;
         E = 0;
-        n_rec = 0;
-        for (uint32_t k = 0; k < ns; k++) {
+        uint32_t k = k_first, i0 = i_first;
+        uint32_t r_cur = pass == 0u && k == 0u ? r_head : load_turn(k, i0);
+        while (k < ns) {
             const uint32_t tile = (uint32_t)__builtin_amdgcn_readlane((int)tile_v, (int)k);
-            uint32_t c = (uint32_t)__builtin_amdgcn_readlane((int)cnt_v, (int)k);
-            c = c < p.rec.seg_len ? c : p.rec.seg_len;
-            const uint32_t *seg = p.rec.rec + ((size_t)q * p.rec.stride + k) * p.rec.seg_len;
-            n_rec += c;
-            for (uint32_t i0 = 0; i0 < c; i0 += 64) {
-                const uint32_t i = i0 + lane;
-                const bool valid = i < c;
-                const uint32_t r = seg[valid ? i : 0u];
-                const uint32_t ref = tile * 8192u + (r & 8191u);
-                uint32_t cnt = r >> 13;
-                cnt = cnt <= tq ? cnt : tq;
-                const uint32_t ch = ref >> 3, j = ref & 7u;
-                const double tv = tz[cnt];
-                const uint32_t rk = p.bnd_rank[ch], bits = p.bnd_bits[ch];
-                const double pv = valid ? tv : 0.0;
-                const uint32_t f = valid ? rk + (uint32_t)__popc(bits & ((1u << j) - 1u)) : 0xFFFFFFFFu;
-                const double incl = carry + wave_incl_scan_f64_dpp(pv);
-                const uint32_t f_next = (uint32_t)__shfl_down((int)f, 1, 64);
-                const bool is_end = valid && (lane == 63u || f_next != f);
-                const unsigned long long em = __ballot(is_end);
-                if (pass == 0u) {
-                    const uint32_t pos = E + (uint32_t)__popcll(em & lt_mask);
-                    if (is_end && pos < kTailEntries) { ent_f[pos] = f; ent_S[pos] = incl; }
-                } else {
-                    const uint32_t f_first = (uint32_t)__builtin_amdgcn_readfirstlane((int)f);
-                    for (uint32_t b = filled + lane; b < f_first; b += 64) Prow[b] = carry;
-                    unsigned long long rest = em;
-                    while (rest) {
-                        const int e = __builtin_ctzll(rest);
-                        rest &= rest - 1ull;
-                        const uint32_t fa = (uint32_t)__builtin_amdgcn_readlane((int)f, e);
-                        const double sa = readlane_f64(incl, e);
-                        if (rest) {
-                            const uint32_t fb = (uint32_t)__builtin_amdgcn_readlane((int)f_next, e);
-                            for (uint32_t b = fa + lane; b < fb; b += 64) Prow[b] = sa;
-                            filled = fb;
-                        } else {
-                            if (lane == 0) Prow[fa] = sa;
-                            filled = fa;
-                        }
+            const uint32_t c = (uint32_t)__builtin_amdgcn_readlane((int)cnt_v, (int)k);
+            uint32_t k_next = k, i_next = i0;
+            advance(k_next, i_next);
+            const uint32_t r_next = load_turn(k_next, i_next);
+            const uint32_t i = i0 + lane;
+            const bool valid = i < c;
+            const uint32_t r = r_cur;
+            const uint32_t ref = tile * 8192u + (r & 8191u);
+            uint32_t cnt = r >> 13;
+            cnt = cnt <= tq ? cnt : tq;
+            const uint32_t ch = ref >> 3, j = ref & 7u;
+            const double tv = tz[cnt];
+            const uint32_t rk = p.bnd_rank[ch], bits = p.bnd_bits[ch];
+            const double pv = valid ? tv : 0.0;
+            const uint32_t f = valid ? rk + (uint32_t)__popc(bits & ((1u << j) - 1u)) : 0xFFFFFFFFu;
+            const double incl = carry + wave_incl_scan_f64_dpp(pv);
+            const uint32_t f_next = (uint32_t)__shfl_down((int)f, 1, 64);
+            const bool is_end = valid && (lane == 63u || f_next != f);
+            const unsigned long long em = __ballot(is_end);
+            if (pass == 0u) {
+                const uint32_t pos = E + (uint32_t)__popcll(em & lt_mask);
+                if (is_end && pos < kTailEntries) { ent_f[pos] = f; ent_S[pos] = incl; }
+            } else {
+                const uint32_t f_first = (uint32_t)__builtin_amdgcn_readfirstlane((int)f);
+                for (uint32_t b = filled + lane; b < f_first; b += 64) Prow[b] = carry;
+                unsigned long long rest = em;
+                while (rest) {
+                    const int e = __builtin_ctzll(rest);
+                    rest &= rest - 1ull;
+                    const uint32_t fa = (uint32_t)__builtin_amdgcn_readlane((int)f, e);
+                    const double sa = readlane_f64(incl, e);
+                    if (rest) {
+                        const uint32_t fb = (uint32_t)__builtin_amdgcn_readlane((int)f_next, e);
+                        for (uint32_t b = fa + lane; b < fb; b += 64) Prow[b] = sa;
+                        filled = fb;
+                    } else {
+                        if (lane == 0) Prow[fa] = sa;
+                        filled = fa;
                     }
                 }
-                E += (uint32_t)__popcll(em);
-                carry = readlane_f64(incl, 63);
             }
+            E += (uint32_t)__popcll(em);
+            carry = readlane_f64(incl, 63);
+            r_cur = r_next;
+            k = k_next;
+            i0 = i_next;
         }
         if (pass == 0u) {
             if (E <= kTailEntries) break;
diff --git a/raxtax_amd/csrc/rtx_wave.hpp b/raxtax_amd/csrc/rtx_wave.hpp
--- a/raxtax_amd/csrc/rtx_wave.hpp
+++ b/raxtax_amd/csrc/rtx_wave.hpp
@@ -7,6 +7,12 @@
 namespace rtx {
 
 __device__ __forceinline__ uint32_t lane_id() { return threadIdx.x & 63u; }
+
+__device__ __forceinline__ uint32_t lane_zero() {
+    uint32_t z;
+    asm("v_mov_b32 %0, 0" : "=v"(z));
+    return z;
+}
 
 __device__ __forceinline__ uint32_t wave_incl_scan_u32(uint32_t v) {
     v += (uint32_t)__builtin_amdgcn_update_dpp(0, (int)v, 0x111, 0xF, 0xF, true);
```
